# facebookresearch/esm

Measured on NVIDIA H100. Metric: sequences/sec ESM-2 650M L=1024 embedding extract, higher is better.
Workload: dtype f16 operands, f32 accumulate/residual/LayerNorm/softmax

## Files before the change

### esm_b200/csrc/api.cu

```cuda
#include "../../include/esmb200.h"

#include <cuda.h>
#include <cuda_runtime.h>
#include <stdio.h>
#include <stdlib.h>
#include <string.h>

#include <string>
#include <vector>

#include <mutex>

#include "attention8.cuh"
#include "attention_contact.cuh"
#include "attention_probs.cuh"
#include "common.cuh"
#include "elementwise.cuh"
#include "gemm2.cuh"
#include "tied_attention.cuh"

using namespace esmb200;

namespace {

thread_local std::string g_last_error;

int fail(int code, const std::string& msg) {
  g_last_error = msg;
  return code;
}

int fail_cuda(cudaError_t e, const char* what) {
  if (e == cudaErrorMemoryAllocation)
    return fail(ESMB200_ENOMEM, std::string("CUDA out of memory. (") + what + ")");
  return fail(ESMB200_ECUDA, std::string(what) + ": " + cudaGetErrorString(e));
}

#define CK(expr)                                        \
  do {                                                  \
    cudaError_t _e = (expr);                            \
    if (_e != cudaSuccess) return fail_cuda(_e, #expr); \
  } while (0)


enum ProfTag : int { T_LN1 = 0, T_QKV, T_ATTN, T_OUT, T_LN2, T_FC1, T_FC2, T_KEYBITS, T_EMBED, T_LN_F32, T_PROBS,
                     T_CONVERT, T_GEMM_OTHER, T_MEANPOOL, T_TIED_SCORES, T_TIED_SOFTMAX, T_TIED_PV, T_COUNT };
struct Profiler {
  std::mutex mu;
  bool on = false;
  std::vector<cudaEvent_t> ev;
  std::vector<int> tag;
  size_t used = 0;
  long long launches = 0;
};
Profiler g_prof;

struct ProfScope {
  cudaStream_t st;
  bool rec;
  size_t slot = 0;
  ProfScope(int tag, cudaStream_t s) : st(s), rec(false) {
    std::lock_guard<std::mutex> lk(g_prof.mu);
    ++g_prof.launches;
    if (g_prof.on && g_prof.used + 2 <= g_prof.ev.size()) {
      rec = true;
      slot = g_prof.used;
      g_prof.used += 2;
      g_prof.tag.push_back(tag);
      cudaEventRecord(g_prof.ev[slot], st);
    }
  }
  ~ProfScope() {
    if (rec) cudaEventRecord(g_prof.ev[slot + 1], st);
  }
};

typedef CUresult (*EncodeTiledFn)(CUtensorMap*, CUtensorMapDataType, cuuint32_t, void*, const cuuint64_t*,
                                  const cuuint64_t*, const cuuint32_t*, const cuuint32_t*, CUtensorMapInterleave,
                                  CUtensorMapSwizzle, CUtensorMapL2promotion, CUtensorMapFloatOOBfill);

EncodeTiledFn get_encode_fn() {
  static EncodeTiledFn fn = nullptr;
  if (fn) return fn;
  void* p = nullptr;
  cudaDriverEntryPointQueryResult qres;
  if (cudaGetDriverEntryPoint("cuTensorMapEncodeTiled", &p, cudaEnableDefault, &qres) != cudaSuccess ||
      qres != cudaDriverEntryPointSuccess)
    return nullptr;
  fn = reinterpret_cast<EncodeTiledFn>(p);
  return fn;
}

int make_tmap_2d(CUtensorMap* map, const void* ptr, int esize, uint64_t rows, uint64_t cols, uint64_t ld_elems,
                 uint32_t box_rows) {
  EncodeTiledFn enc = get_encode_fn();
  if (!enc) return fail(ESMB200_ECUDA, "cuTensorMapEncodeTiled entry point not available");
  if ((reinterpret_cast<uintptr_t>(ptr) & 15) != 0 || (ld_elems * esize) % 16 != 0)
    return fail(ESMB200_EINVAL, "TMA operand must be 16-byte aligned with a 16-byte multiple row pitch");
  cuuint64_t dims[2] = {cols, rows};
  cuuint64_t strides[1] = {ld_elems * (uint64_t)esize};
  cuuint32_t box[2] = {(cuuint32_t)(128 / esize), box_rows};
  cuuint32_t estr[2] = {1, 1};
  CUresult r = enc(map, esize == 2 ? CU_TENSOR_MAP_DATA_TYPE_FLOAT16 : CU_TENSOR_MAP_DATA_TYPE_FLOAT32, 2,
                   const_cast<void*>(ptr), dims, strides, box, estr,
                   CU_TENSOR_MAP_INTERLEAVE_NONE, CU_TENSOR_MAP_SWIZZLE_128B, CU_TENSOR_MAP_L2_PROMOTION_L2_256B,
                   CU_TENSOR_MAP_FLOAT_OOB_FILL_NONE);
  if (r != CUDA_SUCCESS) {
    char buf[160];
    snprintf(buf, sizeof buf, "cuTensorMapEncodeTiled failed (%d) rows=%llu cols=%llu ld=%llu box_rows=%u", (int)r,
             (unsigned long long)rows, (unsigned long long)cols, (unsigned long long)ld_elems, box_rows);
    return fail(ESMB200_ECUDA, buf);
  }
  return ESMB200_OK;
}

int make_tmap_f16(CUtensorMap* map, const void* ptr, uint64_t rows, uint64_t cols, uint64_t ld_elems,
                  uint32_t box_rows) {
  return make_tmap_2d(map, ptr, 2, rows, cols, ld_elems, box_rows);
}

inline int head_slots(int E, int H) { return (H > 0 && E / H > 64) ? 2 : 1; }

constexpr int kMaxDevices = 64;

int num_sms() {
  static int n[kMaxDevices] = {};
  int dev = 0;
  cudaGetDevice(&dev);
  if (dev < 0 || dev >= kMaxDevices) dev = 0;
  if (n[dev] == 0) cudaDeviceGetAttribute(&n[dev], cudaDevAttrMultiProcessorCount, dev);
  return n[dev];
}

int check_device() {
  static int ok[kMaxDevices] = {};
  int dev = 0;
  if (cudaGetDevice(&dev) != cudaSuccess) return fail(ESMB200_ECUDA, "no CUDA device");
  if (dev < 0 || dev >= kMaxDevices) return fail(ESMB200_ECUDA, "device ordinal out of range");
  if (ok[dev] == 0) {
    int major = 0;
    cudaDeviceGetAttribute(&major, cudaDevAttrComputeCapabilityMajor, dev);
    ok[dev] = (major == 9) ? 1 : -1;
  }
  if (ok[dev] < 0)
    return fail(ESMB200_ECUDA, "esmb200 requires an sm_90a (Hopper H100) device; there is no fallback path");
  return ESMB200_OK;
}

size_t align_up(size_t v, size_t a) { return (v + a - 1) / a * a; }

int launch_gemm(int epi, const CUtensorMap& ta, const CUtensorMap& tb, const GemmParams& p, cudaStream_t st,
                int tag = T_GEMM_OTHER, bool split = false) {
  ProfScope ps(tag, st);
  cudaError_t e;
  if (split) {
    if (p.K % 64 != 0) return fail(ESMB200_EINVAL, "fp32x3 precision needs K % 64 == 0");
    switch (epi) {
      case EPI_QKV_ROPE: e = launch_gemm2_epi<EPI_QKV_ROPE, true>(ta, tb, p, num_sms(), st); break;
      case EPI_BIAS_RESIDUAL: e = launch_gemm2_epi<EPI_BIAS_RESIDUAL, true>(ta, tb, p, num_sms(), st); break;
      case EPI_BIAS_GELU: e = launch_gemm2_epi<EPI_BIAS_GELU, true>(ta, tb, p, num_sms(), st); break;
      case EPI_BIAS_F32: e = launch_gemm2_epi<EPI_BIAS_F32, true>(ta, tb, p, num_sms(), st); break;
      case EPI_BIAS_GELU_F32: e = launch_gemm2_epi<EPI_BIAS_GELU_F32, true>(ta, tb, p, num_sms(), st); break;
      default: return fail(ESMB200_EINVAL, "unknown GEMM epilogue");
    }
    if (e != cudaSuccess) return fail_cuda(e, "gemm launch (fp32x3)");
    return ESMB200_OK;
  }
  switch (epi) {
    case EPI_QKV_ROPE: e = launch_gemm2_epi<EPI_QKV_ROPE>(ta, tb, p, num_sms(), st); break;
    case EPI_BIAS_RESIDUAL: e = launch_gemm2_epi<EPI_BIAS_RESIDUAL>(ta, tb, p, num_sms(), st); break;
    case EPI_BIAS_GELU: e = launch_gemm2_epi<EPI_BIAS_GELU>(ta, tb, p, num_sms(), st); break;
    case EPI_BIAS_F32: e = launch_gemm2_epi<EPI_BIAS_F32>(ta, tb, p, num_sms(), st); break;
    case EPI_BIAS_GELU_F32: e = launch_gemm2_epi<EPI_BIAS_GELU_F32>(ta, tb, p, num_sms(), st); break;
    default: return fail(ESMB200_EINVAL, "unknown GEMM epilogue");
  }
  if (e != cudaSuccess) return fail_cuda(e, "gemm launch");
  return ESMB200_OK;
}

struct AttnScratch {
  uint32_t* keybits;
  int* kvlen;
  float* row_max;
  float* row_sum;
  int words;
};

size_t attn_scratch_bytes(int B, int T, int H) {
  const int words = (int)align_up((size_t)(T + 31) / 32, 4);
  return align_up((size_t)B * words * 4, 256) + align_up((size_t)B * 4, 256) + 2 * align_up((size_t)B * H * T * 4, 256);
}

AttnScratch carve_attn_scratch(void* scratch, int B, int T, int H) {
  AttnScratch s;
  s.words = (int)align_up((size_t)(T + 31) / 32, 4);
  uint8_t* p = static_cast<uint8_t*>(scratch);
  s.keybits = reinterpret_cast<uint32_t*>(p);
  p += align_up((size_t)B * s.words * 4, 256);
  s.kvlen = reinterpret_cast<int*>(p);
  p += align_up((size_t)B * 4, 256);
  s.row_max = reinterpret_cast<float*>(p);
  p += align_up((size_t)B * H * T * 4, 256);
  s.row_sum = reinterpret_cast<float*>(p);
  return s;
}

int run_key_bits(const uint8_t* pad_mask, const AttnScratch& s, int B, int T, cudaStream_t st) {
  const int wpb = 4;
  ProfScope ps(T_KEYBITS, st);
  key_bits_kernel<<<(B + wpb - 1) / wpb, wpb * 32, 0, st>>>(pad_mask, s.keybits, s.kvlen, B, T, s.words);
  CK(cudaGetLastError());
  return ESMB200_OK;
}

struct ContactLayer {
  const float* w;
  const uint8_t* keep;
  float* acc;
  float* row_part;
  float* col_part;
  int lo, S;
};

int run_attention(const void* qkv, void* ctx, float* probs, long long probs_batch_stride, int attn_flags,
                  const AttnScratch& s, int B, int T, int H, cudaStream_t st, bool split = false,
                  const ContactLayer* contact = nullptr, int slots = 1) {
  const int E = H * 64 * slots;
  if (slots == 2 && split) return fail(ESMB200_EINVAL, "head_dim > 64: fp32x3 precision is not available");
  const uint64_t qcols = (uint64_t)(split ? 6 : 3) * E;
  CUtensorMap tq;
  int rc = make_tmap_f16(&tq, qkv, (uint64_t)B * T, qcols, qcols, 128);
  if (rc) return rc;
  AttnParams ap;
  ap.B = B; ap.T = T; ap.H = H; ap.E = E;
  ap.lo_off = split ? 3 * E : 0;
  ap.slots = slots;
  ap.keybits = s.keybits; ap.kvlen = s.kvlen; ap.words = s.words;
  ap.ctx = static_cast<__half*>(ctx);
  ap.row_max = probs ? s.row_max : nullptr;
  ap.row_sum = probs ? s.row_sum : nullptr;
  cudaError_t e;
  {
    CUtensorMap tkv;
    rc = make_tmap_f16(&tkv, qkv, (uint64_t)B * T, qcols, qcols, attn8_cfg::BLOCK_KV);
    if (rc) return rc;
    ProfScope ps(T_ATTN, st);
    e = launch_attention_fwd(tq, tkv, ap, st);
  }
  if (e != cudaSuccess) return fail_cuda(e, "attention launch");
  if (probs && contact && !split) {
    if (B > 65535) return fail(ESMB200_EINVAL, "return_contacts: B must be <= 65535");
    ContactFuseParams cp;
    cp.B = B; cp.T = T; cp.H = H; cp.E = E; cp.slots = slots;
    cp.keybits = s.keybits; cp.kvlen = s.kvlen; cp.words = s.words;
    cp.row_max = s.row_max; cp.row_sum = s.row_sum; cp.probs = probs;
    cp.batch_stride = probs_batch_stride > 0 ? probs_batch_stride : (long long)H * T * T;
    cp.zero_pad_rows = attn_flags & 1;
    cp.w = contact->w; cp.keep = contact->keep; cp.acc = contact->acc;
    cp.row_part = contact->row_part; cp.col_part = contact->col_part; cp.lo = contact->lo; cp.S = contact->S;
    {
      ProfScope ps(T_PROBS, st);
      e = launch_attention_probs_contact(tq, cp, st);
    }
    if (e != cudaSuccess) return fail_cuda(e, "attention probs+contact launch");
    return ESMB200_OK;
  }
  if (probs) {
    if ((size_t)B * H > 65535) return fail(ESMB200_EINVAL, "need_head_weights: B*H must be <= 65535");
    ProbsParams pp;
    pp.B = B; pp.T = T; pp.H = H; pp.E = E;
    pp.keybits = s.keybits; pp.kvlen = s.kvlen; pp.words = s.words;
    pp.row_max = s.row_max; pp.row_sum = s.row_sum; pp.probs = probs;
    pp.batch_stride = probs_batch_stride > 0 ? probs_batch_stride : (long long)H * T * T;
    pp.zero_pad_rows = attn_flags & 1;
    pp.lo_off = split ? 3 * E : 0;
    pp.slots = slots;
    {
      ProfScope ps(T_PROBS, st);
      e = launch_attention_probs(tq, pp, st);
    }
    if (e != cudaSuccess) return fail_cuda(e, "attention probs launch");
  }
  return ESMB200_OK;
}

}

struct esmb200_layer {
  int E, H, F;
  int d;
  int slots;
  int Ea;
  float q_scale;
  int split;
  float eps;
  const float *ln1_w, *ln1_b, *ln2_w, *ln2_b, *out_b, *fc1_b, *fc2_b;
  __half* w_qkv;
  __half* w_out;
  __half* w_fc1;
  __half* w_fc2;
  float* b_qkv;
  CUtensorMap tm_qkv, tm_out, tm_fc1, tm_fc2;
};

extern "C" {

int esmb200_abi_version(void) { return ESMB200_ABI_VERSION; }

const char* esmb200_last_error(void) { return g_last_error.c_str(); }

int esmb200_convert_f16(const float* src, void* dst, size_t n, void* stream) {
  if (n == 0) return ESMB200_OK;
  cudaStream_t st = static_cast<cudaStream_t>(stream);
  size_t blocks = (n + 255) / 256;
  if (blocks > (size_t)num_sms() * 16) blocks = (size_t)num_sms() * 16;
  ProfScope ps(T_CONVERT, st);
  convert_f32_f16_kernel<<<(unsigned)blocks, 256, 0, st>>>(src, static_cast<__half*>(dst), n);
  CK(cudaGetLastError());
  return ESMB200_OK;
}

int esmb200_layer_destroy(esmb200_layer* L) {
  if (!L) return ESMB200_OK;
  cudaFree(L->w_qkv);
  cudaFree(L->w_out);
  cudaFree(L->w_fc1);
  cudaFree(L->w_fc2);
  cudaFree(L->b_qkv);
  delete L;
  return ESMB200_OK;
}

int esmb200_layer_create(const esmb200_layer_weights* w, void* stream, esmb200_layer** out) {
  if (!w || !out) return fail(ESMB200_EINVAL, "null argument");
  int rc = check_device();
  if (rc) return rc;
  const int E = w->embed_dim, H = w->num_heads, F = w->ffn_dim;
  if (E <= 0 || H <= 0 || E % H != 0) return fail(ESMB200_EINVAL, "embed_dim must be a positive multiple of num_heads");
  const int d = w->head_dim > 0 ? w->head_dim : E / H;
  if (d * H != E || d > 128 || d % 2 != 0)
    return fail(ESMB200_EINVAL, "esmb200 supports even head_dim <= 128 (every ESM-2 model, MSA Transformer)");
  if (E % 16 != 0) return fail(ESMB200_EINVAL, "embed_dim must be a multiple of 16");
  const bool has_ffn = w->fc1_weight != nullptr;
  if (has_ffn && (F <= 0 || F % 64 != 0)) return fail(ESMB200_EINVAL, "ffn_dim must be a positive multiple of 64");
  cudaStream_t st = static_cast<cudaStream_t>(stream);
  esmb200_layer* L = new esmb200_layer();
  memset(static_cast<void*>(L), 0, sizeof(*L));
  const int slots = head_slots(E, H);
  const int Ea = 64 * slots * H;
  L->E = E; L->H = H; L->F = has_ffn ? F : 0; L->d = d; L->slots = slots; L->Ea = Ea; L->eps = w->ln_eps;
  L->q_scale = 1.0f / sqrtf((float)d);
  L->ln1_w = w->ln1_weight; L->ln1_b = w->ln1_bias; L->ln2_w = w->ln2_weight; L->ln2_b = w->ln2_bias;
  L->out_b = w->out_bias; L->fc1_b = w->fc1_bias; L->fc2_b = w->fc2_bias;
  if (w->precision != 0 && w->precision != 1) {
    delete L;
    return fail(ESMB200_EINVAL, "precision must be 0 (fp16 operands) or 1 (fp32x3: fp16 hi|lo operands)");
  }
  const int split = w->precision;
  if (split && slots == 2) {
    delete L;
    return fail(ESMB200_EINVAL, "fp32x3 precision is not available for head_dim > 64");
  }
  if (split && (E % 64 != 0 || (has_ffn && F % 64 != 0))) {
    delete L;
    return fail(ESMB200_EINVAL, "fp32x3 precision needs embed_dim % 64 == 0 (all ESM-2 models except 35M)");
  }
  L->split = split;
  const size_t pf = split ? 2 : 1;
  const size_t EaE = (size_t)Ea * E, EF = (size_t)E * F;
  cudaError_t e;
#define ALLOC(ptr, bytes)                                              \
  if ((e = cudaMalloc(reinterpret_cast<void**>(&(ptr)), (bytes))) != cudaSuccess) { \
    esmb200_layer_destroy(L);                                          \
    return fail_cuda(e, "cudaMalloc(packed weights)");                 \
  }
  ALLOC(L->w_qkv, 3 * EaE * 2 * pf);
  ALLOC(L->w_out, EaE * 2 * pf);
  if (has_ffn) {
    ALLOC(L->w_fc1, EF * 2 * pf);
    ALLOC(L->w_fc2, EF * 2 * pf);
  }
  ALLOC(L->b_qkv, (size_t)3 * Ea * 4);
#undef ALLOC
  auto convert = [&](const float* src, __half* dst, size_t rows, int K) -> int {
    if (!split) return esmb200_convert_f16(src, dst, rows * (size_t)K, stream);
    size_t blocks = (rows * (size_t)K + 255) / 256;
    if (blocks > (size_t)num_sms() * 16) blocks = (size_t)num_sms() * 16;
    ProfScope ps(T_CONVERT, st);
    convert_f32_split_kernel<<<(unsigned)blocks, 256, 0, st>>>(src, dst, rows, K);
    cudaError_t ce = cudaGetLastError();
    return ce == cudaSuccess ? ESMB200_OK : fail_cuda(ce, "convert_f32_split");
  };
  if (d == 64 && !split) {
    rc = esmb200_convert_f16(w->q_weight, L->w_qkv, EaE, stream);
    if (!rc) rc = esmb200_convert_f16(w->k_weight, L->w_qkv + EaE, EaE, stream);
    if (!rc) rc = esmb200_convert_f16(w->v_weight, L->w_qkv + 2 * EaE, EaE, stream);
    if (!rc) rc = esmb200_convert_f16(w->out_weight, L->w_out, EaE, stream);
    if (!rc) {
      e = cudaMemcpyAsync(L->b_qkv, w->q_bias, (size_t)E * 4, cudaMemcpyDeviceToDevice, st);
      if (e == cudaSuccess) e = cudaMemcpyAsync(L->b_qkv + E, w->k_bias, (size_t)E * 4, cudaMemcpyDeviceToDevice, st);
      if (e == cudaSuccess) e = cudaMemcpyAsync(L->b_qkv + 2 * E, w->v_bias, (size_t)E * 4, cudaMemcpyDeviceToDevice, st);
      if (e != cudaSuccess) rc = fail_cuda(e, "bias pack");
    }
  } else {
    e = cudaMemsetAsync(L->w_qkv, 0, 3 * EaE * 2 * pf, st);
    if (e == cudaSuccess) e = cudaMemsetAsync(L->w_out, 0, EaE * 2 * pf, st);
    if (e == cudaSuccess) e = cudaMemsetAsync(L->b_qkv, 0, (size_t)3 * Ea * 4, st);
    if (e != cudaSuccess) rc = fail_cuda(e, "memset(packed weights)");
    const float* ws3[3] = {w->q_weight, w->k_weight, w->v_weight};
    const float* bs3[3] = {w->q_bias, w->k_bias, w->v_bias};
    const unsigned blocks = (unsigned)(((size_t)E * E + 255) / 256);
    for (int s3 = 0; s3 < 3 && !rc; ++s3) {
      ProfScope ps(T_CONVERT, st);
      pack_head_rows_kernel<<<blocks, 256, 0, st>>>(ws3[s3], bs3[s3], L->w_qkv + (size_t)s3 * EaE * pf, L->b_qkv + s3 * Ea,
                                                    E, d, split);
      if ((e = cudaGetLastError()) != cudaSuccess) rc = fail_cuda(e, "pack_head_rows");
    }
    if (!rc) {
      ProfScope ps(T_CONVERT, st);
      pack_head_cols_kernel<<<blocks, 256, 0, st>>>(w->out_weight, L->w_out, E, Ea, d, split);
      if ((e = cudaGetLastError()) != cudaSuccess) rc = fail_cuda(e, "pack_head_cols");
    }
  }
  if (!rc && has_ffn) rc = convert(w->fc1_weight, L->w_fc1, F, E);
  if (!rc && has_ffn) rc = convert(w->fc2_weight, L->w_fc2, E, F);
  const uint32_t wbox = gemm2_cfg::HALF_N;
  if (!rc) rc = make_tmap_f16(&L->tm_qkv, L->w_qkv, 3 * (uint64_t)Ea, pf * E, pf * E, wbox);
  if (!rc) rc = make_tmap_f16(&L->tm_out, L->w_out, E, pf * Ea, pf * Ea, wbox);
  if (!rc && has_ffn) rc = make_tmap_f16(&L->tm_fc1, L->w_fc1, F, pf * E, pf * E, wbox);
  if (!rc && has_ffn) rc = make_tmap_f16(&L->tm_fc2, L->w_fc2, E, pf * F, pf * F, wbox);
  if (rc) {
    esmb200_layer_destroy(L);
    return rc;
  }
  *out = L;
  return ESMB200_OK;
}

size_t esmb200_attention_scratch_bytes(int32_t B, int32_t T) {
  return attn_scratch_bytes(B, T, 64);
}

size_t esmb200_workspace_bytes(int32_t E, int32_t H, int32_t F, int32_t B, int32_t T, int32_t precision) {
  const size_t M = (size_t)B * T, Ea = (size_t)64 * head_slots(E, H) * H, pf = precision ? 2 : 1;
  const size_t a = align_up(M * E * 2 * pf, 1024);
  const size_t big_qkv_ctx = align_up(M * 3 * Ea * 2 * pf, 1024) + align_up(M * Ea * 2 * pf, 1024);
  const size_t big_h = align_up(M * F * 2 * pf, 1024);
  const size_t big = big_qkv_ctx > big_h ? big_qkv_ctx : big_h;
  return a + big + attn_scratch_bytes(B, T, H) + 1024;
}

namespace {
struct Workspace {
  __half* xn;
  __half* qkv;
  __half* ctx;
  __half* h;
  AttnScratch as;
};

int carve_workspace(Workspace* ws, void* workspace, size_t bytes, int E, int H, int F, int B, int T, int split) {
  if (bytes < esmb200_workspace_bytes(E, H, F, B, T, split)) return fail(ESMB200_EWORKSPACE, "workspace too small");
  const size_t M = (size_t)B * T, Ea = (size_t)64 * head_slots(E, H) * H, pf = split ? 2 : 1;
  uint8_t* p = reinterpret_cast<uint8_t*>(align_up(reinterpret_cast<uintptr_t>(workspace), 1024));
  ws->xn = reinterpret_cast<__half*>(p);
  p += align_up(M * E * 2 * pf, 1024);
  ws->qkv = reinterpret_cast<__half*>(p);
  ws->h = reinterpret_cast<__half*>(p);
  ws->ctx = reinterpret_cast<__half*>(p + align_up(M * 3 * Ea * 2 * pf, 1024));
  const size_t big_qkv_ctx = align_up(M * 3 * Ea * 2 * pf, 1024) + align_up(M * Ea * 2 * pf, 1024);
  const size_t big_h = align_up(M * F * 2 * pf, 1024);
  p += big_qkv_ctx > big_h ? big_qkv_ctx : big_h;
  ws->as = carve_attn_scratch(p, B, T, H);
  return ESMB200_OK;
}

struct ActMaps {
  CUtensorMap xn, ctx, h;
};

int layer_forward_impl(esmb200_layer* L, float* x, int B, int T, const float* rope_cos, const float* rope_sin,
                       float* attn_probs, long long attn_batch_stride, int attn_flags, const Workspace& ws,
                       const ActMaps& am, cudaStream_t st, const ContactLayer* contact = nullptr) {
  const int E = L->E, F = L->F, H = L->H, Ea = L->Ea;
  const int M = B * T;
  const bool split = L->split != 0;
  cudaError_t e = cudaSuccess;
  {
    ProfScope ps(T_LN1, st);
    e = split ? launch_layernorm<2>(x, L->ln1_w, L->ln1_b, ws.xn, M, E, L->eps, st)
              : launch_layernorm<1>(x, L->ln1_w, L->ln1_b, ws.xn, M, E, L->eps, st);
  }
  if (e != cudaSuccess) return fail_cuda(e, "layernorm1");
  GemmParams g;
  memset(&g, 0, sizeof g);
  g.M = M; g.N = 3 * Ea; g.K = E; g.bias = L->b_qkv; g.out = ws.qkv; g.ldo = 3 * Ea;
  g.rope_cos = rope_cos; g.rope_sin = rope_sin; g.T = T; g.E = Ea; g.q_scale = L->q_scale;
  g.lo_col_off = 3 * Ea;
  g.rope_ld = 32 * L->slots;
  int rc = launch_gemm(EPI_QKV_ROPE, am.xn, L->tm_qkv, g, st, T_QKV, split);
  if (rc) return rc;
  rc = run_attention(ws.qkv, ws.ctx, attn_probs, attn_batch_stride, attn_flags, ws.as, B, T, H, st, split, contact,
                     L->slots);
  if (rc) return rc;
  memset(&g, 0, sizeof g);
  g.M = M; g.N = E; g.K = Ea; g.bias = L->out_b; g.out = x; g.ldo = E;
  rc = launch_gemm(EPI_BIAS_RESIDUAL, am.ctx, L->tm_out, g, st, T_OUT, split);
  if (rc) return rc;
  {
    ProfScope ps(T_LN2, st);
    e = split ? launch_layernorm<2>(x, L->ln2_w, L->ln2_b, ws.xn, M, E, L->eps, st)
              : launch_layernorm<1>(x, L->ln2_w, L->ln2_b, ws.xn, M, E, L->eps, st);
  }
  if (e != cudaSuccess) return fail_cuda(e, "layernorm2");
  memset(&g, 0, sizeof g);
  g.M = M; g.N = F; g.K = E; g.bias = L->fc1_b; g.out = ws.h; g.ldo = F; g.lo_col_off = F;
  rc = launch_gemm(EPI_BIAS_GELU, am.xn, L->tm_fc1, g, st, T_FC1, split);
  if (rc) return rc;
  memset(&g, 0, sizeof g);
  g.M = M; g.N = E; g.K = F; g.bias = L->fc2_b; g.out = x; g.ldo = E;
  rc = launch_gemm(EPI_BIAS_RESIDUAL, am.h, L->tm_fc2, g, st, T_FC2, split);
  return rc;
}

int make_act_maps(ActMaps* am, const Workspace& ws, int E, int H, int F, int M, int split = 0) {
  const uint64_t Ea = (uint64_t)64 * head_slots(E, H) * H, pf = split ? 2 : 1;
  int rc = make_tmap_f16(&am->xn, ws.xn, M, pf * E, pf * E, gemm2_cfg::BOX_M);
  if (!rc) rc = make_tmap_f16(&am->ctx, ws.ctx, M, pf * Ea, pf * Ea, gemm2_cfg::BOX_M);
  if (!rc) rc = make_tmap_f16(&am->h, ws.h, M, pf * F, pf * F, gemm2_cfg::BOX_M);
  return rc;
}
}

int esmb200_stack_forward(esmb200_layer* const* layers, int32_t n_layers, float* x, const uint8_t* pad_mask,
                          int32_t B, int32_t T, const float* rope_cos, const float* rope_sin,
                          float* const* repr_out, float* const* attn_out, int64_t attn_batch_stride,
                          int32_t attn_flags, const esmb200_contact_job* contact, void* workspace,
                          size_t workspace_bytes, void* stream) {
  if (!layers || n_layers <= 0 || !x || !rope_cos || !rope_sin || !workspace)
    return fail(ESMB200_EINVAL, "null argument");
  if (contact) {
    if (!attn_out) return fail(ESMB200_EINVAL, "a contact job needs attn_out for every layer");
    for (int i = 0; i < n_layers; ++i)
      if (!attn_out[i]) return fail(ESMB200_EINVAL, "a contact job needs attn_out for every layer");
    if (!contact->weights || !contact->acc || !contact->row_part || !contact->col_part || contact->lo < 0 ||
        contact->hi > T || contact->hi <= contact->lo)
      return fail(ESMB200_EINVAL, "bad contact job");
  }
  if (B <= 0 || T <= 0) return fail(ESMB200_EINVAL, "empty batch");
  if ((long long)B * T > 0x7fffffffLL / 8) return fail(ESMB200_EINVAL, "B*T too large for one call; split the batch");
  int rc = check_device();
  if (rc) return rc;
  cudaStream_t st = static_cast<cudaStream_t>(stream);
  const int E = layers[0]->E, F = layers[0]->F, H = layers[0]->H;
  if (F <= 0) return fail(ESMB200_EINVAL, "attention-only layers belong to esmb200_axial_stack_forward");
  for (int i = 1; i < n_layers; ++i)
    if (layers[i]->E != E || layers[i]->F != F || layers[i]->H != H || layers[i]->split != layers[0]->split)
      return fail(ESMB200_EINVAL, "layers of one stack must share E, H, F and precision");
  const int split = layers[0]->split;
  Workspace ws;
  rc = carve_workspace(&ws, workspace, workspace_bytes, E, H, F, B, T, split);
  if (rc) return rc;
  ActMaps am;
  rc = make_act_maps(&am, ws, E, H, F, B * T, split);
  if (rc) return rc;
  rc = run_key_bits(pad_mask, ws.as, B, T, st);
  if (rc) return rc;
  const int nt128 = (T + 127) / 128;
  for (int i = 0; i < n_layers; ++i) {
    ContactLayer cl;
    if (contact) {
      const int S = contact->hi - contact->lo;
      const size_t part = (size_t)B * H * nt128 * S;
      cl.w = contact->weights + (size_t)i * H; cl.keep = contact->keep; cl.acc = contact->acc;
      cl.row_part = contact->row_part + (size_t)i * 4 * part; cl.col_part = contact->col_part + (size_t)i * 4 * part;
      cl.lo = contact->lo; cl.S = S;
    }
    rc = layer_forward_impl(layers[i], x, B, T, rope_cos, rope_sin, attn_out ? attn_out[i] : nullptr, attn_batch_stride,
                            attn_flags, ws, am, st, contact ? &cl : nullptr);
    if (rc) return rc;
    if (repr_out && repr_out[i])
      CK(cudaMemcpyAsync(repr_out[i], x, (size_t)B * T * E * 4, cudaMemcpyDeviceToDevice, st));
  }
  return ESMB200_OK;
}

int esmb200_layer_forward(esmb200_layer* layer, float* x, const uint8_t* pad_mask, int32_t B, int32_t T,
                          const float* rope_cos, const float* rope_sin, float* attn_probs, void* workspace,
                          size_t workspace_bytes, void* stream) {
  if (!layer) return fail(ESMB200_EINVAL, "null layer");
  float* attn_arr[1] = {attn_probs};
  esmb200_layer* arr[1] = {layer};
  return esmb200_stack_forward(arr, 1, x, pad_mask, B, T, rope_cos, rope_sin, nullptr, attn_probs ? attn_arr : nullptr,
                               0, 0, nullptr, workspace, workspace_bytes, stream);
}

int esmb200_embed_tokens(const int64_t* tokens, const float* table, float* x, int32_t B, int32_t T, int32_t E,
                         int32_t padding_idx, int32_t mask_idx, int32_t token_dropout, void* stream) {
  if (!tokens || !table || !x) return fail(ESMB200_EINVAL, "null argument");
  if (B <= 0 || B > 65535 || T <= 0 || E % 4 != 0) return fail(ESMB200_EINVAL, "bad shape");
  ProfScope ps(T_EMBED, static_cast<cudaStream_t>(stream));
  int chunks = (8 * num_sms() + B - 1) / B;
  if (chunks > (T + 3) / 4) chunks = (T + 3) / 4;
  if (chunks < 1) chunks = 1;
  embed_tokens_kernel<<<dim3(chunks, B), 256, 0, static_cast<cudaStream_t>(stream)>>>(tokens, table, x, T, E, padding_idx,
                                                                                     mask_idx, token_dropout);
  CK(cudaGetLastError());
  return ESMB200_OK;
}

int esmb200_layernorm(const float* x, const float* weight, const float* bias, float* out, int32_t M, int32_t E,
                      float eps, void* stream) {
  if (!x || !weight || !bias || !out) return fail(ESMB200_EINVAL, "null argument");
  ProfScope ps(T_LN_F32, static_cast<cudaStream_t>(stream));
  cudaError_t e = launch_layernorm<0>(x, weight, bias, out, M, E, eps, static_cast<cudaStream_t>(stream));
  if (e != cudaSuccess) return fail_cuda(e, "layernorm");
  return ESMB200_OK;
}

int esmb200_layernorm_f16(const float* x, const float* weight, const float* bias, void* out, int32_t M, int32_t E,
                          float eps, void* stream) {
  if (!x || !weight || !bias || !out) return fail(ESMB200_EINVAL, "null argument");
  ProfScope ps(T_LN1, static_cast<cudaStream_t>(stream));
  cudaError_t e = launch_layernorm<1>(x, weight, bias, out, M, E, eps, static_cast<cudaStream_t>(stream));
  if (e != cudaSuccess) return fail_cuda(e, "layernorm_f16");
  return ESMB200_OK;
}

int esmb200_gemm_f16(int32_t epilogue, const void* a, const void* w, const float* bias, void* out, int32_t M,
                     int32_t N, int32_t K, const float* rope_cos, const float* rope_sin, int32_t T, int32_t E,
                     void* stream) {
  if (!a || !w || !bias || !out) return fail(ESMB200_EINVAL, "null argument");
  const bool f16_out = (epilogue == EPI_QKV_ROPE || epilogue == EPI_BIAS_GELU);
  if (M <= 0 || N <= 0 || K <= 0 || K % 8 != 0 || N % (f16_out ? 64 : 32) != 0)
    return fail(ESMB200_EINVAL, "gemm needs K % 8 == 0 and N % 64 == 0 (fp16 output) / N % 32 == 0 (fp32 output)");
  int rc = check_device();
  if (rc) return rc;
  if (epilogue == EPI_QKV_ROPE && (!rope_cos || !rope_sin || T <= 0 || E <= 0 || E % 64 != 0 || N != 3 * E))
    return fail(ESMB200_EINVAL, "qkv epilogue needs rope tables, T and N == 3E");
  CUtensorMap ta, tb;
  rc = make_tmap_f16(&ta, a, M, K, K, gemm2_cfg::BOX_M);
  if (!rc) rc = make_tmap_f16(&tb, w, N, K, K, gemm2_cfg::HALF_N);
  if (rc) return rc;
  GemmParams g;
  memset(&g, 0, sizeof g);
  g.M = M; g.N = N; g.K = K; g.bias = bias; g.out = out; g.ldo = N;
  g.rope_cos = rope_cos; g.rope_sin = rope_sin; g.T = T; g.E = E; g.q_scale = 0.125f;
  return launch_gemm(epilogue, ta, tb, g, static_cast<cudaStream_t>(stream));
}

int esmb200_layernorm_split(const float* x, const float* weight, const float* bias, void* out, int32_t M, int32_t E,
                            float eps, void* stream) {
  if (!x || !weight || !bias || !out) return fail(ESMB200_EINVAL, "null argument");
  ProfScope ps(T_LN1, static_cast<cudaStream_t>(stream));
  cudaError_t e = launch_layernorm<2>(x, weight, bias, out, M, E, eps, static_cast<cudaStream_t>(stream));
  if (e != cudaSuccess) return fail_cuda(e, "layernorm_split");
  return ESMB200_OK;
}

int esmb200_convert_split(const float* src, void* dst, int64_t rows, int32_t K, void* stream) {
  if (!src || !dst) return fail(ESMB200_EINVAL, "null argument");
  if (rows <= 0 || K <= 0) return ESMB200_OK;
  cudaStream_t st = static_cast<cudaStream_t>(stream);
  size_t blocks = ((size_t)rows * K + 255) / 256;
  if (blocks > (size_t)num_sms() * 16) blocks = (size_t)num_sms() * 16;
  ProfScope ps(T_CONVERT, st);
  convert_f32_split_kernel<<<(unsigned)blocks, 256, 0, st>>>(src, static_cast<__half*>(dst), (size_t)rows, K);
  CK(cudaGetLastError());
  return ESMB200_OK;
}

int esmb200_gemm_split(int32_t epilogue, const void* a, const void* w, const float* bias, void* out, int32_t M,
                       int32_t N, int32_t K, const float* rope_cos, const float* rope_sin, int32_t T, int32_t E,
                       void* stream) {
  if (!a || !w || !bias || !out) return fail(ESMB200_EINVAL, "null argument");
  const bool f16_out = (epilogue == EPI_QKV_ROPE || epilogue == EPI_BIAS_GELU);
  if (M <= 0 || N <= 0 || K <= 0 || K % 64 != 0 || N % (f16_out ? 64 : 32) != 0)
    return fail(ESMB200_EINVAL, "split gemm needs K % 64 == 0 and N % 64 == 0 (fp16 output) / N % 32 == 0 (fp32 output)");
  if (epilogue < 0 || epilogue > EPI_BIAS_GELU_F32) return fail(ESMB200_EINVAL, "unknown GEMM epilogue");
  int rc = check_device();
  if (rc) return rc;
  if (epilogue == EPI_QKV_ROPE && (!rope_cos || !rope_sin || T <= 0 || E <= 0 || E % 64 != 0 || N != 3 * E))
    return fail(ESMB200_EINVAL, "qkv epilogue needs rope tables, T and N == 3E");
  CUtensorMap ta, tb;
  rc = make_tmap_f16(&ta, a, M, 2 * (uint64_t)K, 2 * (uint64_t)K, gemm2_cfg::BOX_M);
  if (!rc) rc = make_tmap_f16(&tb, w, N, 2 * (uint64_t)K, 2 * (uint64_t)K, gemm2_cfg::HALF_N);
  if (rc) return rc;
  GemmParams g;
  memset(&g, 0, sizeof g);
  g.M = M; g.N = N; g.K = K; g.bias = bias; g.out = out; g.ldo = N; g.lo_col_off = N;
  g.rope_cos = rope_cos; g.rope_sin = rope_sin; g.T = T; g.E = E; g.q_scale = 0.125f;
  return launch_gemm(epilogue, ta, tb, g, static_cast<cudaStream_t>(stream), T_GEMM_OTHER, true);
}

int esmb200_attention_split(const void* qkv, const uint8_t* pad_mask, void* ctx, float* attn_probs, int32_t B, int32_t T,
                            int32_t H, void* scratch, void* stream) {
  if (!qkv || !ctx || !scratch) return fail(ESMB200_EINVAL, "null argument");
  if (B <= 0 || T <= 0 || H <= 0 || H > 64) return fail(ESMB200_EINVAL, "bad shape");
  int rc = check_device();
  if (rc) return rc;
  cudaStream_t st = static_cast<cudaStream_t>(stream);
  AttnScratch s = carve_attn_scratch(scratch, B, T, H);
  rc = run_key_bits(pad_mask, s, B, T, st);
  if (rc) return rc;
  return run_attention(qkv, ctx, attn_probs, 0, 0, s, B, T, H, st, true);
}

int esmb200_gemm_qkv_f16(const void* a, const void* w, const float* bias, void* out, int32_t M, int32_t E, float q_scale,
                         const float* rope_cos, const float* rope_sin, int32_t T, void* stream) {
  if (!a || !w || !bias || !out) return fail(ESMB200_EINVAL, "null argument");
  if (M <= 0 || E <= 0 || E % 64 != 0) return fail(ESMB200_EINVAL, "qkv gemm needs E % 64 == 0");
  if ((rope_cos == nullptr) != (rope_sin == nullptr) || (rope_cos && T <= 0))
    return fail(ESMB200_EINVAL, "rope tables must be given together with T, or not at all");
  int rc = check_device();
  if (rc) return rc;
  CUtensorMap ta, tb;
  rc = make_tmap_f16(&ta, a, M, E, E, gemm2_cfg::BOX_M);
  if (!rc) rc = make_tmap_f16(&tb, w, 3 * (uint64_t)E, E, E, gemm2_cfg::HALF_N);
  if (rc) return rc;
  GemmParams g;
  memset(&g, 0, sizeof g);
  g.M = M; g.N = 3 * E; g.K = E; g.bias = bias; g.out = out; g.ldo = 3 * E;
  g.rope_cos = rope_cos; g.rope_sin = rope_sin; g.T = T > 0 ? T : 1; g.E = E; g.q_scale = q_scale;
  return launch_gemm(EPI_QKV_ROPE, ta, tb, g, static_cast<cudaStream_t>(stream));
}

int esmb200_attention(const void* qkv, const uint8_t* pad_mask, void* ctx, float* attn_probs, int32_t B, int32_t T,
                      int32_t H, void* scratch, void* stream) {
  if (!qkv || !ctx || !scratch) return fail(ESMB200_EINVAL, "null argument");
  if (B <= 0 || T <= 0 || H <= 0 || H > 64) return fail(ESMB200_EINVAL, "bad shape");
  int rc = check_device();
  if (rc) return rc;
  cudaStream_t st = static_cast<cudaStream_t>(stream);
  AttnScratch s = carve_attn_scratch(scratch, B, T, H);
  rc = run_key_bits(pad_mask, s, B, T, st);
  if (rc) return rc;
  return run_attention(qkv, ctx, attn_probs, 0, 0, s, B, T, H, st);
}

int esmb200_attention128(const void* qkv, const uint8_t* pad_mask, void* ctx, float* attn_probs, int32_t B, int32_t T,
                         int32_t H, void* scratch, void* stream) {
  if (!qkv || !ctx || !scratch) return fail(ESMB200_EINVAL, "null argument");
  if (B <= 0 || T <= 0 || H <= 0 || H > 64) return fail(ESMB200_EINVAL, "bad shape");
  int rc = check_device();
  if (rc) return rc;
  cudaStream_t st = static_cast<cudaStream_t>(stream);
  AttnScratch s = carve_attn_scratch(scratch, B, T, H);
  rc = run_key_bits(pad_mask, s, B, T, st);
  if (rc) return rc;
  return run_attention(qkv, ctx, attn_probs, 0, 0, s, B, T, H, st, false, nullptr, 2);
}

size_t esmb200_tied_row_attention_scratch_bytes(int32_t B, int32_t C, int32_t H) {
  const size_t Cp = align_up((size_t)C, 64);
  return align_up((size_t)H * B * C * C * 4, 1024) + align_up((size_t)H * B * C * Cp * 2, 1024) + 2048;
}

static int tied_row_impl(const void* qkv, const uint8_t* key_pad, long long key_pad_stride, void* ctx,
                         float* attn_probs, int32_t B, int32_t R, int32_t C, int32_t H, void* scratch,
                         size_t scratch_bytes, void* stream) {
  if (!qkv || !ctx || !scratch) return fail(ESMB200_EINVAL, "null argument");
  if (B <= 0 || R <= 0 || C <= 0 || H <= 0 || H > 64 || (long long)B * H > 65535)
    return fail(ESMB200_EINVAL, "bad shape");
  if (C > TIED_MAX_C) return fail(ESMB200_EINVAL, "tied row attention supports at most 1024 alignment columns");
  if (scratch_bytes < esmb200_tied_row_attention_scratch_bytes(B, C, H))
    return fail(ESMB200_EWORKSPACE, "tied row attention scratch too small");
  int rc = check_device();
  if (rc) return rc;
  cudaStream_t st = static_cast<cudaStream_t>(stream);
  const int E = H * 64;
  const size_t Cp = align_up((size_t)C, 64);
  uint8_t* sp = reinterpret_cast<uint8_t*>(align_up(reinterpret_cast<uintptr_t>(scratch), 1024));
  TiedParams tp;
  tp.B = B; tp.R = R; tp.C = C; tp.H = H; tp.E = E; tp.Cp = (int)Cp;
  tp.S = attn_probs ? attn_probs : reinterpret_cast<float*>(sp);
  tp.P = reinterpret_cast<__half*>(sp + align_up((size_t)H * B * C * C * 4, 1024));
  tp.ctx = static_cast<__half*>(ctx);
  tp.key_pad = key_pad;
  tp.key_pad_stride = key_pad_stride;
  tp.write_probs = attn_probs ? 1 : 0;
  const uint64_t rows = (uint64_t)B * R * C;
  CUtensorMap tq, tk, tv, tpm;
  if ((rc = make_tmap_f16(&tq, qkv, rows, (uint64_t)3 * E, (uint64_t)3 * E, tied_cfg::S_BM))) return rc;
  if ((rc = make_tmap_f16(&tk, qkv, rows, (uint64_t)3 * E, (uint64_t)3 * E, tied_cfg::S_BN))) return rc;
  if ((rc = make_tmap_f16(&tv, qkv, rows, (uint64_t)3 * E, (uint64_t)3 * E, 64))) return rc;
  if ((rc = make_tmap_f16(&tpm, tp.P, (uint64_t)H * B * C, Cp, Cp, tied_cfg::V_BM))) return rc;
  cudaError_t e;
  {
    ProfScope ps(T_TIED_SCORES, st);
    e = launch_tied_scores(tq, tk, tp, st);
  }
  if (e != cudaSuccess) return fail_cuda(e, "tied scores launch");
  {
    ProfScope ps(T_TIED_SOFTMAX, st);
    e = launch_tied_softmax(tp, st);
  }
  if (e != cudaSuccess) return fail_cuda(e, "tied softmax launch");
  {
    ProfScope ps(T_TIED_PV, st);
    e = launch_tied_pv(tpm, tv, tp, st);
  }
  if (e != cudaSuccess) return fail_cuda(e, "tied update launch");
  return ESMB200_OK;
}

int esmb200_tied_row_attention(const void* qkv, const uint8_t* key_pad, void* ctx, float* attn_probs, int32_t B,
                               int32_t R, int32_t C, int32_t H, void* scratch, size_t scratch_bytes, void* stream) {
  return tied_row_impl(qkv, key_pad, C, ctx, attn_probs, B, R, C, H, scratch, scratch_bytes, stream);
}

int esmb200_column_attention(const void* qkv, const uint8_t* pad_mask, void* ctx, int32_t B, int32_t R, int32_t C,
                             int32_t H, void* scratch, void* stream) {
  if (!qkv || !ctx || !scratch) return fail(ESMB200_EINVAL, "null argument");
  if (B <= 0 || R <= 0 || C <= 0 || H <= 0 || H > 64) return fail(ESMB200_EINVAL, "bad shape");
  int rc = check_device();
  if (rc) return rc;
  cudaStream_t st = static_cast<cudaStream_t>(stream);
  const int E = H * 64;
  const int S = B * C;
  AttnScratch s = carve_attn_scratch(scratch, S, R, H);
  rc = run_key_bits(pad_mask, s, S, R, st);
  if (rc) return rc;
  CUtensorMap tq, tkv;
  const uint64_t wide = (uint64_t)C * 3 * E;
  if ((rc = make_tmap_f16(&tq, qkv, (uint64_t)B * R, wide, wide, attn8_cfg::BLOCK_Q))) return rc;
  if ((rc = make_tmap_f16(&tkv, qkv, (uint64_t)B * R, wide, wide, attn8_cfg::BLOCK_KV))) return rc;
  AttnParams ap;
  ap.B = S; ap.T = R; ap.H = H; ap.E = E;
  ap.keybits = s.keybits; ap.kvlen = s.kvlen; ap.words = s.words;
  ap.ctx = static_cast<__half*>(ctx);
  ap.row_max = nullptr; ap.row_sum = nullptr;
  ap.cols = C;
  cudaError_t e;
  {
    ProfScope ps(T_ATTN, st);
    e = launch_attention_fwd(tq, tkv, ap, st);
  }
  if (e != cudaSuccess) return fail_cuda(e, "column attention launch");
  return ESMB200_OK;
}


size_t esmb200_axial_workspace_bytes(int32_t E, int32_t F, int32_t B, int32_t R, int32_t C) {
  return esmb200_workspace_bytes(E, E / 64, F, B * C, R, 0) + esmb200_tied_row_attention_scratch_bytes(B, C, E / 64) + 1024;
}

int esmb200_axial_stack_forward(esmb200_layer* const* row_layers, esmb200_layer* const* col_layers, int32_t n_layers,
                                float* x, const uint8_t* pad_mask, const uint8_t* col_pad_mask, int32_t B, int32_t R,
                                int32_t C, float* const* row_attn_out, void* workspace, size_t workspace_bytes,
                                void* stream) {
  if (!row_layers || !col_layers || n_layers <= 0 || !x || !workspace) return fail(ESMB200_EINVAL, "null argument");
  if (B <= 0 || R <= 0 || C <= 0) return fail(ESMB200_EINVAL, "empty alignment");
  if ((pad_mask == nullptr) != (col_pad_mask == nullptr))
    return fail(ESMB200_EINVAL, "pad_mask [B,R,C] and col_pad_mask [B,C,R] must be given together");
  if ((long long)B * R * C > 0x7fffffffLL / 8) return fail(ESMB200_EINVAL, "B*R*C too large for one call");
  int rc = check_device();
  if (rc) return rc;
  cudaStream_t st = static_cast<cudaStream_t>(stream);
  const int E = col_layers[0]->E, F = col_layers[0]->F, H = col_layers[0]->H;
  if (F <= 0) return fail(ESMB200_EINVAL, "col_layers carry the feed-forward weights");
  for (int i = 0; i < n_layers; ++i)
    if (row_layers[i]->E != E || col_layers[i]->E != E || col_layers[i]->F != F)
      return fail(ESMB200_EINVAL, "layers of one stack must share E and F");
  if (workspace_bytes < esmb200_axial_workspace_bytes(E, F, B, R, C))
    return fail(ESMB200_EWORKSPACE, "workspace too small");
  const int M = B * R * C;
  Workspace ws;
  if (E != 64 * H) return fail(ESMB200_EINVAL, "the MSA axial path needs head_dim 64");
  for (int i = 0; i < n_layers; ++i)
    if (row_layers[i]->split || col_layers[i]->split)
      return fail(ESMB200_EINVAL, "the MSA axial path runs with fp16 operands only (precision 0)");
  const size_t base_bytes = esmb200_workspace_bytes(E, H, F, B * C, R, 0);
  rc = carve_workspace(&ws, workspace, base_bytes, E, H, F, B * C, R, 0);
  if (rc) return rc;
  uint8_t* tied_scratch = reinterpret_cast<uint8_t*>(align_up(reinterpret_cast<uintptr_t>(workspace), 1024)) + base_bytes;
  const size_t tied_bytes = esmb200_tied_row_attention_scratch_bytes(B, C, H);
  ActMaps am;
  rc = make_act_maps(&am, ws, E, H, F, M);
  if (rc) return rc;
  rc = run_key_bits(col_pad_mask, ws.as, B * C, R, st);
  if (rc) return rc;
  CUtensorMap tcq, tckv;
  const uint64_t wide = (uint64_t)C * 3 * E;
  if ((rc = make_tmap_f16(&tcq, ws.qkv, (uint64_t)B * R, wide, wide, attn8_cfg::BLOCK_Q))) return rc;
  if ((rc = make_tmap_f16(&tckv, ws.qkv, (uint64_t)B * R, wide, wide, attn8_cfg::BLOCK_KV))) return rc;
  const float row_scale = 0.125f / sqrtf((float)R);
  cudaError_t e;
  GemmParams g;
  for (int i = 0; i < n_layers; ++i) {
    esmb200_layer* L = row_layers[i];
    {
      ProfScope ps(T_LN1, st);
      e = launch_layernorm<1>(x, L->ln1_w, L->ln1_b, ws.xn, M, E, L->eps, st);
    }
    if (e != cudaSuccess) return fail_cuda(e, "row layernorm");
    memset(&g, 0, sizeof g);
    g.M = M; g.N = 3 * E; g.K = E; g.bias = L->b_qkv; g.out = ws.qkv; g.ldo = 3 * E;
    g.T = 1; g.E = E; g.q_scale = row_scale;
    rc = launch_gemm(EPI_QKV_ROPE, am.xn, L->tm_qkv, g, st, T_QKV);
    if (rc) return rc;
    if (pad_mask) {
      ProfScope ps(T_KEYBITS, st);
      zero_q_at_pads_kernel<<<(M + 7) / 8, 256, 0, st>>>(ws.qkv, pad_mask, M, E);
      CK(cudaGetLastError());
    }
    rc = tied_row_impl(ws.qkv, pad_mask, (long long)R * C, ws.ctx, row_attn_out ? row_attn_out[i] : nullptr, B, R, C, H,
                       tied_scratch, tied_bytes, stream);
    if (rc) return rc;
    memset(&g, 0, sizeof g);
    g.M = M; g.N = E; g.K = E; g.bias = L->out_b; g.out = x; g.ldo = E;
    rc = launch_gemm(EPI_BIAS_RESIDUAL, am.ctx, L->tm_out, g, st, T_OUT);
    if (rc) return rc;
    L = col_layers[i];
    {
      ProfScope ps(T_LN1, st);
      e = launch_layernorm<1>(x, L->ln1_w, L->ln1_b, ws.xn, M, E, L->eps, st);
    }
    if (e != cudaSuccess) return fail_cuda(e, "column layernorm");
    memset(&g, 0, sizeof g);
    g.M = M; g.N = 3 * E; g.K = E; g.bias = L->b_qkv; g.out = ws.qkv; g.ldo = 3 * E;
    g.T = 1; g.E = E; g.q_scale = 0.125f;
    rc = launch_gemm(EPI_QKV_ROPE, am.xn, L->tm_qkv, g, st, T_QKV);
    if (rc) return rc;
    {
      AttnParams ap;
      ap.B = B * C; ap.T = R; ap.H = H; ap.E = E;
      ap.keybits = ws.as.keybits; ap.kvlen = ws.as.kvlen; ap.words = ws.as.words;
      ap.ctx = ws.ctx; ap.row_max = nullptr; ap.row_sum = nullptr; ap.cols = C;
      ProfScope ps(T_ATTN, st);
      e = launch_attention_fwd(tcq, tckv, ap, st);
    }
    if (e != cudaSuccess) return fail_cuda(e, "column attention launch");
    memset(&g, 0, sizeof g);
    g.M = M; g.N = E; g.K = E; g.bias = L->out_b; g.out = x; g.ldo = E;
    rc = launch_gemm(EPI_BIAS_RESIDUAL, am.ctx, L->tm_out, g, st, T_OUT);
    if (rc) return rc;
    {
      ProfScope ps(T_LN2, st);
      e = launch_layernorm<1>(x, L->ln2_w, L->ln2_b, ws.xn, M, E, L->eps, st);
    }
    if (e != cudaSuccess) return fail_cuda(e, "ffn layernorm");
    memset(&g, 0, sizeof g);
    g.M = M; g.N = F; g.K = E; g.bias = L->fc1_b; g.out = ws.h; g.ldo = F;
    rc = launch_gemm(EPI_BIAS_GELU, am.xn, L->tm_fc1, g, st, T_FC1);
    if (rc) return rc;
    memset(&g, 0, sizeof g);
    g.M = M; g.N = E; g.K = F; g.bias = L->fc2_b; g.out = x; g.ldo = E;
    rc = launch_gemm(EPI_BIAS_RESIDUAL, am.h, L->tm_fc2, g, st, T_FC2);
    if (rc) return rc;
  }
  return ESMB200_OK;
}



int esmb200_msa_embed(const int64_t* tokens, const float* embed_table, const float* pos_table, const float* msa_pos,
                      int32_t msa_pos_dim, const float* ln_weight, const float* ln_bias, float eps, float* x,
                      int32_t B, int32_t R, int32_t C, int32_t E, int32_t padding_idx, void* stream) {
  if (!tokens || !embed_table || !pos_table || !ln_weight || !ln_bias || !x) return fail(ESMB200_EINVAL, "null argument");
  if (B <= 0 || R <= 0 || C <= 0 || E <= 0 || E % 4 != 0 || E > 20 * 128) return fail(ESMB200_EINVAL, "bad shape");
  if (msa_pos && msa_pos_dim != E && msa_pos_dim != 1)
    return fail(ESMB200_EINVAL, "msa_position_embedding width must be E or 1");
  cudaStream_t st = static_cast<cudaStream_t>(stream);
  ProfScope ps(T_EMBED, st);
  const size_t smem = (size_t)C * sizeof(int);
  const int grid = B * R;
  if (E <= 4 * 128)
    msa_embed_kernel<4><<<grid, 256, smem, st>>>(tokens, embed_table, pos_table, msa_pos, msa_pos_dim, ln_weight,
                                                  ln_bias, eps, x, R, C, E, padding_idx);
  else if (E <= 10 * 128)
    msa_embed_kernel<10><<<grid, 256, smem, st>>>(tokens, embed_table, pos_table, msa_pos, msa_pos_dim, ln_weight,
                                                   ln_bias, eps, x, R, C, E, padding_idx);
  else
    msa_embed_kernel<20><<<grid, 256, smem, st>>>(tokens, embed_table, pos_table, msa_pos, msa_pos_dim, ln_weight,
                                                   ln_bias, eps, x, R, C, E, padding_idx);
  CK(cudaGetLastError());
  return ESMB200_OK;
}


int esmb200_contact_accumulate(const float* attn, int64_t batch_stride, const float* w, const uint8_t* keep, float* acc,
                               float* row_sum, float* col_part, int32_t B, int32_t H, int32_t T, int32_t lo, int32_t hi,
                               void* stream) {
  if (!attn || !w || !acc || !row_sum || !col_part) return fail(ESMB200_EINVAL, "null argument");
  const int S = hi - lo;
  if (B <= 0 || H <= 0 || T <= 0 || lo < 0 || hi > T || S <= 0 || B > 65535) return fail(ESMB200_EINVAL, "bad shape");
  if (S > 1024) return fail(ESMB200_EINVAL, "contact head supports at most 1024 positions");
  cudaStream_t st = static_cast<cudaStream_t>(stream);
  ProfScope ps(T_PROBS, st);
  const size_t smem = (size_t)8 * S * sizeof(float);
  dim3 grid((S + 15) / 16, B);
  if (S <= 512)
    contact_accumulate_kernel<2, 16, 2><<<grid, 256, smem, st>>>(attn, batch_stride, w, keep, acc, row_sum, col_part, H, T,
                                                                  lo, S);
  else
    contact_accumulate_kernel<2, 32, 1><<<grid, 256, smem, st>>>(attn, batch_stride, w, keep, acc, row_sum, col_part, H, T,
                                                                  lo, S);
  CK(cudaGetLastError());
  return ESMB200_OK;
}

int esmb200_contact_finalize(const float* acc, const float* u, const float* a1, const float* bias, float* out, int32_t B,
                             int32_t C, int32_t S, void* stream) {
  if (!acc || !u || !a1 || !out) return fail(ESMB200_EINVAL, "null argument");
  if (B <= 0 || C <= 0 || S <= 0 || B > 65535) return fail(ESMB200_EINVAL, "bad shape");
  cudaStream_t st = static_cast<cudaStream_t>(stream);
  ProfScope ps(T_PROBS, st);
  dim3 grid((S + 63) / 64, (S + 63) / 64, B);
  contact_finalize_kernel<<<grid, 256, 0, st>>>(acc, u, a1, bias, out, C, S);
  CK(cudaGetLastError());
  return ESMB200_OK;
}


int esmb200_mean_pool(const float* x, const int32_t* lengths, float* out, int32_t B, int32_t T, int32_t E,
                      void* stream) {
  if (!x || !lengths || !out) return fail(ESMB200_EINVAL, "null argument");
  if (B <= 0 || T < 2 || E <= 0 || B > 65535) return fail(ESMB200_EINVAL, "bad shape");
  cudaStream_t st = static_cast<cudaStream_t>(stream);
  ProfScope ps(T_MEANPOOL, st);
  if (E % 4 != 0) return fail(ESMB200_EINVAL, "mean_pool needs E % 4 == 0");
  dim3 grid((E + 127) / 128, B);
  mean_pool_kernel<<<grid, 256, 0, st>>>(x, lengths, out, T, E);
  CK(cudaGetLastError());
  return ESMB200_OK;
}


int esmb200_set_option(const char* name, int32_t value) {
  if (!name) return fail(ESMB200_EINVAL, "null option name");
  if (!strcmp(name, "pdl") && (value == 0 || value == 1)) { pdl_flag() = value; return ESMB200_OK; }
  return fail(ESMB200_EINVAL, std::string("unknown option or value: ") + name);
}

long long esmb200_launch_count(void) {
  std::lock_guard<std::mutex> lk(g_prof.mu);
  return g_prof.launches;
}

int esmb200_profile_enable(int32_t max_launches) {
  std::lock_guard<std::mutex> lk(g_prof.mu);
  for (cudaEvent_t e : g_prof.ev) cudaEventDestroy(e);
  g_prof.ev.clear();
  g_prof.tag.clear();
  g_prof.used = 0;
  g_prof.on = max_launches > 0;
  for (int i = 0; i < 2 * max_launches; ++i) {
    cudaEvent_t e;
    CK(cudaEventCreate(&e));
    g_prof.ev.push_back(e);
  }
  return ESMB200_OK;
}

int esmb200_profile_read(int32_t* tags, float* ms, int32_t max_records) {
  std::lock_guard<std::mutex> lk(g_prof.mu);
  const int n = (int)(g_prof.used / 2);
  int out = 0;
  for (int i = 0; i < n && out < max_records; ++i, ++out) {
    CK(cudaEventSynchronize(g_prof.ev[2 * i + 1]));
    float t = 0.f;
    CK(cudaEventElapsedTime(&t, g_prof.ev[2 * i], g_prof.ev[2 * i + 1]));
    tags[out] = g_prof.tag[i];
    ms[out] = t;
  }
  g_prof.used = 0;
  g_prof.tag.clear();
  return out;
}

}
```

### esm_b200/csrc/common.cuh

```cuda
#pragma once

#include <cuda.h>
#include <cuda_fp16.h>
#include <cuda_runtime.h>
#include <stdint.h>
#include <stdio.h>
#include <stdlib.h>

#ifndef ESMB200_WATCHDOG
#define ESMB200_WATCHDOG 1
#endif

namespace esmb200 {

constexpr uint32_t kWarp = 32;

__device__ __forceinline__ uint32_t smem_u32(const void* p) {
  return static_cast<uint32_t>(__cvta_generic_to_shared(p));
}

__device__ __forceinline__ uint32_t lane_id() {
  uint32_t r;
  asm volatile("mov.u32 %0, %%laneid;" : "=r"(r));
  return r;
}

__device__ __forceinline__ bool elect_one() {
  uint32_t pred = 0;
  asm volatile(
      "{\n\t"
      ".reg .pred P1;\n\t"
      "elect.sync _|P1, 0xffffffff;\n\t"
      "selp.u32 %0, 1, 0, P1;\n\t"
      "}\n"
      : "=r"(pred));
  return pred != 0;
}

__device__ __forceinline__ void mbar_init(uint64_t* bar, uint32_t count) {
  asm volatile("mbarrier.init.shared::cta.b64 [%0], %1;" ::"r"(smem_u32(bar)), "r"(count) : "memory");
}

__device__ __forceinline__ void fence_barrier_init() {
  asm volatile("fence.mbarrier_init.release.cluster;" ::: "memory");
}

__device__ __forceinline__ void fence_proxy_async_smem() {
  asm volatile("fence.proxy.async.shared::cta;" ::: "memory");
}

__device__ __forceinline__ void mbar_arrive(uint64_t* bar) {
  asm volatile("mbarrier.arrive.shared::cta.b64 _, [%0];" ::"r"(smem_u32(bar)) : "memory");
}

__device__ __forceinline__ void mbar_arrive_expect_tx(uint64_t* bar, uint32_t bytes) {
  asm volatile("mbarrier.arrive.expect_tx.shared::cta.b64 _, [%0], %1;" ::"r"(smem_u32(bar)), "r"(bytes)
               : "memory");
}

__device__ __forceinline__ bool mbar_try_wait(uint64_t* bar, uint32_t parity) {
  uint32_t ok;
  asm volatile(
      "{\n\t"
      ".reg .pred p;\n\t"
      "mbarrier.try_wait.parity.shared::cta.b64 p, [%1], %2;\n\t"
      "selp.u32 %0, 1, 0, p;\n\t"
      "}\n"
      : "=r"(ok)
      : "r"(smem_u32(bar)), "r"(parity)
      : "memory");
  return ok != 0;
}

__device__ __forceinline__ void mbar_wait(uint64_t* bar, uint32_t parity) {
  if (mbar_try_wait(bar, parity)) return;
#if ESMB200_WATCHDOG
  uint32_t polls = 0;
  while (!mbar_try_wait(bar, parity)) {
    if (++polls == (1u << 26)) {
      printf("esmb200: mbarrier watchdog block=(%d,%d,%d) thread=%d bar=%u parity=%u\n", blockIdx.x, blockIdx.y,
             blockIdx.z, threadIdx.x, smem_u32(bar), parity);
      __trap();
    }
  }
#else
  while (!mbar_try_wait(bar, parity)) {
  }
#endif
}


__device__ __forceinline__ void mbar_wait_relaxed(uint64_t* bar, uint32_t parity) {
  if (mbar_try_wait(bar, parity)) return;
#if ESMB200_WATCHDOG
  uint32_t polls = 0;
#endif
  while (!mbar_try_wait(bar, parity)) {
    __nanosleep(200);
#if ESMB200_WATCHDOG
    if (++polls == (1u << 24)) {
      printf("esmb200: mbarrier watchdog (relaxed) block=(%d,%d,%d) thread=%d bar=%u parity=%u\n", blockIdx.x, blockIdx.y,
             blockIdx.z, threadIdx.x, smem_u32(bar), parity);
      __trap();
    }
#endif
  }
}

__device__ __forceinline__ void tma_prefetch_desc(const CUtensorMap* map) {
  asm volatile("prefetch.tensormap [%0];" ::"l"(reinterpret_cast<uint64_t>(map)) : "memory");
}

__device__ __forceinline__ void tma_load_2d(void* smem_dst, const CUtensorMap* map, uint64_t* bar, int32_t c0,
                                            int32_t c1) {
  asm volatile(
      "cp.async.bulk.tensor.2d.shared::cluster.global.mbarrier::complete_tx::bytes [%0], [%1, {%3, %4}], [%2];"
      :
      : "r"(smem_u32(smem_dst)), "l"(reinterpret_cast<uint64_t>(map)), "r"(smem_u32(bar)), "r"(c0), "r"(c1)
      : "memory");
}

__device__ __forceinline__ void tma_load_2d_addr(uint32_t smem_dst, const CUtensorMap* map, uint32_t bar, int32_t c0,
                                                 int32_t c1) {
  asm volatile(
      "cp.async.bulk.tensor.2d.shared::cluster.global.mbarrier::complete_tx::bytes [%0], [%1, {%3, %4}], [%2];"
      :
      : "r"(smem_dst), "l"(reinterpret_cast<uint64_t>(map)), "r"(bar), "r"(c0), "r"(c1)
      : "memory");
}
__device__ __forceinline__ void mbar_arrive_expect_tx_addr(uint32_t bar, uint32_t bytes) {
  asm volatile("mbarrier.arrive.expect_tx.shared::cta.b64 _, [%0], %1;" ::"r"(bar), "r"(bytes) : "memory");
}

__device__ __forceinline__ void tma_load_2d_hint(void* smem_dst, const CUtensorMap* map, uint64_t* bar, int32_t c0,
                                                 int32_t c1, uint64_t policy) {
  asm volatile(
      "cp.async.bulk.tensor.2d.shared::cluster.global.mbarrier::complete_tx::bytes.L2::cache_hint [%0], [%1, {%3, "
      "%4}], [%2], %5;"
      :
      : "r"(smem_u32(smem_dst)), "l"(reinterpret_cast<uint64_t>(map)), "r"(smem_u32(bar)), "r"(c0), "r"(c1),
        "l"(policy)
      : "memory");
}

__device__ __forceinline__ uint64_t l2_policy_evict_last() {
  uint64_t p;
  asm volatile("createpolicy.fractional.L2::evict_last.b64 %0, 1.0;" : "=l"(p));
  return p;
}
__device__ __forceinline__ uint64_t l2_policy_evict_first() {
  uint64_t p;
  asm volatile("createpolicy.fractional.L2::evict_first.b64 %0, 1.0;" : "=l"(p));
  return p;
}

__device__ __forceinline__ void mma16816(float (&d)[4], const uint32_t (&a)[4], uint32_t b0, uint32_t b1) {
  asm volatile(
      "mma.sync.aligned.m16n8k16.row.col.f32.f16.f16.f32 {%0, %1, %2, %3}, {%4, %5, %6, %7}, {%8, %9}, "
      "{%0, %1, %2, %3};"
      : "+f"(d[0]), "+f"(d[1]), "+f"(d[2]), "+f"(d[3])
      : "r"(a[0]), "r"(a[1]), "r"(a[2]), "r"(a[3]), "r"(b0), "r"(b1));
}

__device__ __forceinline__ void ldsm_x4(uint32_t addr, uint32_t (&r)[4]) {
  asm volatile("ldmatrix.sync.aligned.m8n8.x4.shared.b16 {%0, %1, %2, %3}, [%4];"
               : "=r"(r[0]), "=r"(r[1]), "=r"(r[2]), "=r"(r[3])
               : "r"(addr));
}
__device__ __forceinline__ void ldsm_x4_t(uint32_t addr, uint32_t (&r)[4]) {
  asm volatile("ldmatrix.sync.aligned.m8n8.x4.trans.shared.b16 {%0, %1, %2, %3}, [%4];"
               : "=r"(r[0]), "=r"(r[1]), "=r"(r[2]), "=r"(r[3])
               : "r"(addr));
}

__device__ __forceinline__ uint32_t sw128(uint32_t base, uint32_t row, uint32_t chunk) {
  return base + row * 128u + ((chunk ^ (row & 7u)) << 4);
}

__device__ __forceinline__ void ldsm_a(uint32_t base, uint32_t r0, uint32_t kk, uint32_t (&a)[4]) {
  const uint32_t l = lane_id();
  ldsm_x4(sw128(base, r0 + (l & 15u), 2u * kk + (l >> 4)), a);
}
__device__ __forceinline__ void ldsm_b(uint32_t base, uint32_t n0, uint32_t kk, uint32_t (&b)[4]) {
  const uint32_t l = lane_id();
  ldsm_x4(sw128(base, n0 + (l & 7u) + ((l >> 4) << 3), 2u * kk + ((l >> 3) & 1u)), b);
}
__device__ __forceinline__ void ldsm_bt(uint32_t base, uint32_t kk, uint32_t n0, uint32_t (&b)[4]) {
  const uint32_t l = lane_id();
  ldsm_x4_t(sw128(base, 16u * kk + (l & 15u), n0 / 8u + (l >> 4)), b);
}

__device__ __forceinline__ uint64_t wgmma_desc_sw128(uint32_t smem_addr) {
  uint64_t d = 0;
  d |= static_cast<uint64_t>((smem_addr & 0x3FFFFu) >> 4);
  d |= static_cast<uint64_t>(1) << 16;
  d |= static_cast<uint64_t>(1024 >> 4) << 32;
  d |= static_cast<uint64_t>(1) << 62;
  return d;
}

__device__ __forceinline__ void wgmma_fence() { asm volatile("wgmma.fence.sync.aligned;" ::: "memory"); }
__device__ __forceinline__ void wgmma_commit() { asm volatile("wgmma.commit_group.sync.aligned;" ::: "memory"); }
template <int N>
__device__ __forceinline__ void wgmma_wait() {
  asm volatile("wgmma.wait_group.sync.aligned %0;" ::"n"(N) : "memory");
}
template <int N>
__device__ __forceinline__ void reg_fence_f(float (&r)[N]) {
#pragma unroll
  for (int i = 0; i < N; ++i) asm volatile("" : "+f"(r[i])::"memory");
}

__device__ __forceinline__ void wgmma_m64n256k16(float (&d)[128], uint64_t da, uint64_t db, int scale_d) {
  asm volatile(
      "{\n.reg .pred p;\nsetp.ne.b32 p, %130, 0;\n"
      "wgmma.mma_async.sync.aligned.m64n256k16.f32.f16.f16 "
      "{%0, %1, %2, %3, %4, %5, %6, %7, %8, %9, %10, %11, %12, %13, %14, %15, "
      "%16, %17, %18, %19, %20, %21, %22, %23, %24, %25, %26, %27, %28, %29, %30, %31, "
      "%32, %33, %34, %35, %36, %37, %38, %39, %40, %41, %42, %43, %44, %45, %46, %47, "
      "%48, %49, %50, %51, %52, %53, %54, %55, %56, %57, %58, %59, %60, %61, %62, %63, "
      "%64, %65, %66, %67, %68, %69, %70, %71, %72, %73, %74, %75, %76, %77, %78, %79, "
      "%80, %81, %82, %83, %84, %85, %86, %87, %88, %89, %90, %91, %92, %93, %94, %95, "
      "%96, %97, %98, %99, %100, %101, %102, %103, %104, %105, %106, %107, %108, %109, %110, %111, "
      "%112, %113, %114, %115, %116, %117, %118, %119, %120, %121, %122, %123, %124, %125, %126, %127}, "
      "%128, %129, p, 1, 1, 0, 0;\n}\n"
      : "+f"(d[0]), "+f"(d[1]), "+f"(d[2]), "+f"(d[3]), "+f"(d[4]), "+f"(d[5]), "+f"(d[6]), "+f"(d[7]),
        "+f"(d[8]), "+f"(d[9]), "+f"(d[10]), "+f"(d[11]), "+f"(d[12]), "+f"(d[13]), "+f"(d[14]), "+f"(d[15]),
        "+f"(d[16]), "+f"(d[17]), "+f"(d[18]), "+f"(d[19]), "+f"(d[20]), "+f"(d[21]), "+f"(d[22]), "+f"(d[23]),
        "+f"(d[24]), "+f"(d[25]), "+f"(d[26]), "+f"(d[27]), "+f"(d[28]), "+f"(d[29]), "+f"(d[30]), "+f"(d[31]),
        "+f"(d[32]), "+f"(d[33]), "+f"(d[34]), "+f"(d[35]), "+f"(d[36]), "+f"(d[37]), "+f"(d[38]), "+f"(d[39]),
        "+f"(d[40]), "+f"(d[41]), "+f"(d[42]), "+f"(d[43]), "+f"(d[44]), "+f"(d[45]), "+f"(d[46]), "+f"(d[47]),
        "+f"(d[48]), "+f"(d[49]), "+f"(d[50]), "+f"(d[51]), "+f"(d[52]), "+f"(d[53]), "+f"(d[54]), "+f"(d[55]),
        "+f"(d[56]), "+f"(d[57]), "+f"(d[58]), "+f"(d[59]), "+f"(d[60]), "+f"(d[61]), "+f"(d[62]), "+f"(d[63]),
        "+f"(d[64]), "+f"(d[65]), "+f"(d[66]), "+f"(d[67]), "+f"(d[68]), "+f"(d[69]), "+f"(d[70]), "+f"(d[71]),
        "+f"(d[72]), "+f"(d[73]), "+f"(d[74]), "+f"(d[75]), "+f"(d[76]), "+f"(d[77]), "+f"(d[78]), "+f"(d[79]),
        "+f"(d[80]), "+f"(d[81]), "+f"(d[82]), "+f"(d[83]), "+f"(d[84]), "+f"(d[85]), "+f"(d[86]), "+f"(d[87]),
        "+f"(d[88]), "+f"(d[89]), "+f"(d[90]), "+f"(d[91]), "+f"(d[92]), "+f"(d[93]), "+f"(d[94]), "+f"(d[95]),
        "+f"(d[96]), "+f"(d[97]), "+f"(d[98]), "+f"(d[99]), "+f"(d[100]), "+f"(d[101]), "+f"(d[102]), "+f"(d[103]),
        "+f"(d[104]), "+f"(d[105]), "+f"(d[106]), "+f"(d[107]), "+f"(d[108]), "+f"(d[109]), "+f"(d[110]), "+f"(d[111]),
        "+f"(d[112]), "+f"(d[113]), "+f"(d[114]), "+f"(d[115]), "+f"(d[116]), "+f"(d[117]), "+f"(d[118]), "+f"(d[119]),
        "+f"(d[120]), "+f"(d[121]), "+f"(d[122]), "+f"(d[123]), "+f"(d[124]), "+f"(d[125]), "+f"(d[126]), "+f"(d[127])
      : "l"(da), "l"(db), "r"(scale_d));
}

template <uint32_t R>
__device__ __forceinline__ void setmaxnreg_dec() { asm volatile("setmaxnreg.dec.sync.aligned.u32 %0;" ::"n"(R)); }
template <uint32_t R>
__device__ __forceinline__ void setmaxnreg_inc() { asm volatile("setmaxnreg.inc.sync.aligned.u32 %0;" ::"n"(R)); }

__device__ __forceinline__ void tma_store_2d(const CUtensorMap* map, const void* smem_src, int32_t c0, int32_t c1) {
  asm volatile("cp.async.bulk.tensor.2d.global.shared::cta.bulk_group [%0, {%2, %3}], [%1];" ::"l"(
                   reinterpret_cast<uint64_t>(map)),
               "r"(smem_u32(smem_src)), "r"(c0), "r"(c1)
               : "memory");
}
__device__ __forceinline__ void tma_reduce_add_2d(const CUtensorMap* map, const void* smem_src, int32_t c0,
                                                  int32_t c1) {
  asm volatile("cp.reduce.async.bulk.tensor.2d.global.shared::cta.add.tile.bulk_group [%0, {%2, %3}], [%1];" ::"l"(
                   reinterpret_cast<uint64_t>(map)),
               "r"(smem_u32(smem_src)), "r"(c0), "r"(c1)
               : "memory");
}
__device__ __forceinline__ void tma_store_commit() { asm volatile("cp.async.bulk.commit_group;" ::: "memory"); }
template <int N>
__device__ __forceinline__ void tma_store_wait_read() {
  asm volatile("cp.async.bulk.wait_group.read %0;" ::"n"(N) : "memory");
}
__device__ __forceinline__ void tma_store_wait_all() { asm volatile("cp.async.bulk.wait_group 0;" ::: "memory"); }

__device__ __forceinline__ void pdl_wait() { asm volatile("griddepcontrol.wait;" ::: "memory"); }
__device__ __forceinline__ void pdl_launch_dependents() { asm volatile("griddepcontrol.launch_dependents;" ::: "memory"); }

inline int& pdl_flag() {
  static int flag = -1;
  return flag;
}
inline bool pdl_enabled() {
  int& f = pdl_flag();
  if (f < 0) {
    const char* e = getenv("ESMB200_PDL");
    f = (e && e[0] == '1') ? 1 : 0;
  }
  return f != 0;
}

template <typename... KArgs, typename... Args>
inline cudaError_t launch_pdl(void (*kernel)(KArgs...), dim3 grid, dim3 block, size_t smem, cudaStream_t stream,
                              Args&&... args) {
  cudaLaunchConfig_t cfg = {};
  cfg.gridDim = grid;
  cfg.blockDim = block;
  cfg.dynamicSmemBytes = smem;
  cfg.stream = stream;
  cudaLaunchAttribute attr[1];
  attr[0].id = cudaLaunchAttributeProgrammaticStreamSerialization;
  attr[0].val.programmaticStreamSerializationAllowed = 1;
  cfg.attrs = attr;
  cfg.numAttrs = pdl_enabled() ? 1 : 0;
  return cudaLaunchKernelEx(&cfg, kernel, KArgs(args)...);
}

__device__ __forceinline__ uint32_t pack_half2(float lo, float hi) {
  __half2 h = __floats2half2_rn(lo, hi);
  return *reinterpret_cast<uint32_t*>(&h);
}

__device__ __forceinline__ void fma2(float& d0, float& d1, float a0, float a1, float b0, float b1, float c0, float c1) {
  d0 = fmaf(a0, b0, c0);
  d1 = fmaf(a1, b1, c1);
}
__device__ __forceinline__ void add2(float& d0, float& d1, float a0, float a1, float b0, float b1) {
  d0 = a0 + b0;
  d1 = a1 + b1;
}
__device__ __forceinline__ void mul2(float& d0, float& d1, float a0, float a1, float b0, float b1) {
  d0 = a0 * b0;
  d1 = a1 * b1;
}

__device__ __forceinline__ float ex2_approx(float x) {
  float y;
  asm("ex2.approx.ftz.f32 %0, %1;" : "=f"(y) : "f"(x));
  return y;
}

__device__ __forceinline__ float warp_sum(float v) {
#pragma unroll
  for (int o = 16; o > 0; o >>= 1) v += __shfl_xor_sync(0xffffffffu, v, o);
  return v;
}

__device__ __forceinline__ void named_bar_sync(uint32_t id, uint32_t nthreads) {
  asm volatile("bar.sync %0, %1;" ::"r"(id), "r"(nthreads) : "memory");
}

}
```

### esm_b200/csrc/gemm2.cuh

```cuda
#pragma once

#include "gemm_common.cuh"

namespace esmb200 {

namespace gemm2_cfg {
constexpr int BLOCK_M = 128;
constexpr int BLOCK_N = 256;
constexpr int HALF_N = 128;
constexpr int BLOCK_K = 64;
constexpr int STAGES = 4;
constexpr int A_STAGE_BYTES = BLOCK_M * BLOCK_K * 2;
constexpr int B_STAGE_BYTES = BLOCK_N * BLOCK_K * 2;
constexpr int STAGE_BYTES = A_STAGE_BYTES + B_STAGE_BYTES;
constexpr int BOX_M = 128;
constexpr int NUM_THREADS = 384;
constexpr int SMEM_BYTES = STAGES * STAGE_BYTES + 1024 + 256;
}

template <int EPI, bool SPLIT = false>
__global__ void __launch_bounds__(gemm2_cfg::NUM_THREADS, 1)
gemm2_f16_kernel(const __grid_constant__ CUtensorMap tmap_a, const __grid_constant__ CUtensorMap tmap_b,
                 const GemmParams p) {
  using namespace gemm2_cfg;
  extern __shared__ uint8_t smem_raw[];
  uint8_t* smem = reinterpret_cast<uint8_t*>((reinterpret_cast<uintptr_t>(smem_raw) + 1023) & ~uintptr_t(1023));
  uint8_t* smem_a = smem;
  uint8_t* smem_b = smem + STAGES * A_STAGE_BYTES;
  uint64_t* bars = reinterpret_cast<uint64_t*>(smem + STAGES * STAGE_BYTES);
  uint64_t* full_bar = bars;
  uint64_t* empty_bar = bars + STAGES;

  const uint32_t wg = __shfl_sync(0xffffffffu, threadIdx.x / 128, 0);
  const int tiles_m = (p.M + BLOCK_M - 1) / BLOCK_M;
  const int tiles_n = (p.N + BLOCK_N - 1) / BLOCK_N;
  const int num_tiles = tiles_m * tiles_n;
  const int num_kb1 = (p.K + BLOCK_K - 1) / BLOCK_K;
  const int num_kb = SPLIT ? 3 * num_kb1 : num_kb1;

  if (threadIdx.x == 0) {
    tma_prefetch_desc(&tmap_a);
    tma_prefetch_desc(&tmap_b);
    for (int i = 0; i < STAGES; ++i) {
      mbar_init(&full_bar[i], 1);
      mbar_init(&empty_bar[i], 2);
    }
    fence_barrier_init();
  }
  __syncthreads();
  pdl_launch_dependents();
  pdl_wait();

  if (wg == 0) {
    setmaxnreg_dec<40>();
    if (threadIdx.x == 0) {
      uint32_t it = 0;
      for (int tile = blockIdx.x; tile < num_tiles; tile += gridDim.x) {
        const int m0 = (tile / tiles_n) * BLOCK_M, n0 = (tile % tiles_n) * BLOCK_N;
        for (int kb = 0; kb < num_kb; ++kb, ++it) {
          const uint32_t s = it % STAGES;
          while (!mbar_try_wait(&empty_bar[s], ((it / STAGES) & 1) ^ 1)) __nanosleep(64);
          int a_col = kb * BLOCK_K, b_col = kb * BLOCK_K;
          if constexpr (SPLIT) {
            const int part = kb % 3;
            a_col = (kb / 3) * BLOCK_K + (part == 1 ? p.K : 0);
            b_col = (kb / 3) * BLOCK_K + (part == 2 ? p.K : 0);
          }
          mbar_arrive_expect_tx(&full_bar[s], STAGE_BYTES);
          tma_load_2d(smem_a + s * A_STAGE_BYTES, &tmap_a, &full_bar[s], a_col, m0);
          tma_load_2d(smem_b + s * B_STAGE_BYTES, &tmap_b, &full_bar[s], b_col, n0);
          tma_load_2d(smem_b + s * B_STAGE_BYTES + HALF_N * 128, &tmap_b, &full_bar[s], b_col, n0 + HALF_N);
        }
      }
    }
    return;
  }

  setmaxnreg_inc<232>();
  const uint32_t mw = wg - 1;
  const uint32_t warp = (threadIdx.x / 32) % 4;
  const uint32_t lane = threadIdx.x % 32;
  const uint32_t g = lane / 4, c = lane % 4;
  const bool signal = (threadIdx.x % 128) == 0;
  const uint32_t a_base = smem_u32(smem_a) + mw * 64 * 128;
  const uint32_t b_base = smem_u32(smem_b);
  const size_t pitch = (SPLIT && (EPI == EPI_QKV_ROPE || EPI == EPI_BIAS_GELU)) ? 2 * (size_t)p.ldo : (size_t)p.ldo;
  uint32_t it = 0;
  float acc[128];

  for (int tile = blockIdx.x; tile < num_tiles; tile += gridDim.x) {
    const int m0 = (tile / tiles_n) * BLOCK_M, n0 = (tile % tiles_n) * BLOCK_N;
    for (int kb = 0; kb < num_kb; ++kb, ++it) {
      const uint32_t s = it % STAGES;
      while (!mbar_try_wait(&full_bar[s], (it / STAGES) & 1)) {
      }
      wgmma_fence();
      const uint64_t da = wgmma_desc_sw128(a_base + s * A_STAGE_BYTES);
      const uint64_t db = wgmma_desc_sw128(b_base + s * B_STAGE_BYTES);
#pragma unroll
      for (int k = 0; k < BLOCK_K / 16; ++k) wgmma_m64n256k16(acc, da + 2 * k, db + 2 * k, (kb | k) != 0);
      wgmma_commit();
      wgmma_wait<1>();
      if (kb > 0 && signal) mbar_arrive(&empty_bar[(it + STAGES - 1) % STAGES]);
    }
    wgmma_wait<0>();
    reg_fence_f(acc);
    if (signal) mbar_arrive(&empty_bar[(it + STAGES - 1) % STAGES]);

    const int r0 = m0 + (int)(mw * 64 + warp * 16 + g);
    const int rows[2] = {r0, r0 + 8};
    if constexpr (EPI == EPI_QKV_ROPE) {
      const bool rope = p.rope_cos != nullptr;
      const int ld = p.rope_ld == 64 ? 64 : 32;
#pragma unroll
      for (int gi = 0; gi < 4; ++gi) {
        const int col0 = n0 + gi * 64;
        if (col0 >= p.N) break;
        const int sect = col0 / p.E;
        const float sc = (sect == 0) ? p.q_scale : 1.0f;
        const int slot = p.rope_ld == 64 ? ((col0 >> 6) & 1) : 0;
#pragma unroll
        for (int hr = 0; hr < 2; ++hr) {
          const int row = rows[hr];
          if (row >= p.M) continue;
          const int t = row % p.T;
          __half* o = reinterpret_cast<__half*>(p.out) + (size_t)row * pitch;
#pragma unroll
          for (int q = 0; q < 4; ++q) {
            const int j = 8 * q + 2 * (int)c;
            const float2 bl = __ldg(reinterpret_cast<const float2*>(p.bias + col0 + j));
            const float2 bh = __ldg(reinterpret_cast<const float2*>(p.bias + col0 + 32 + j));
            float a0 = (acc[4 * (8 * gi + q) + 2 * hr] + bl.x) * sc, a1 = (acc[4 * (8 * gi + q) + 2 * hr + 1] + bl.y) * sc;
            float b0 = (acc[4 * (8 * gi + q + 4) + 2 * hr] + bh.x) * sc;
            float b1 = (acc[4 * (8 * gi + q + 4) + 2 * hr + 1] + bh.y) * sc;
            if (sect < 2 && rope) {
              const float2 cs = __ldg(reinterpret_cast<const float2*>(p.rope_cos + (size_t)t * ld + slot * 32 + j));
              const float2 sn = __ldg(reinterpret_cast<const float2*>(p.rope_sin + (size_t)t * ld + slot * 32 + j));
              const float ra0 = a0 * cs.x - b0 * sn.x, rb0 = b0 * cs.x + a0 * sn.x;
              const float ra1 = a1 * cs.y - b1 * sn.y, rb1 = b1 * cs.y + a1 * sn.y;
              a0 = ra0; b0 = rb0; a1 = ra1; b1 = rb1;
            }
            const __half2 ha = __floats2half2_rn(a0, a1), hb = __floats2half2_rn(b0, b1);
            *reinterpret_cast<__half2*>(o + col0 + j) = ha;
            *reinterpret_cast<__half2*>(o + col0 + 32 + j) = hb;
            if constexpr (SPLIT) {
              const float2 fa = __half22float2(ha), fb = __half22float2(hb);
              *reinterpret_cast<__half2*>(o + p.lo_col_off + col0 + j) = __floats2half2_rn(a0 - fa.x, a1 - fa.y);
              *reinterpret_cast<__half2*>(o + p.lo_col_off + col0 + 32 + j) = __floats2half2_rn(b0 - fb.x, b1 - fb.y);
            }
          }
        }
      }
    } else {
#pragma unroll
      for (int i = 0; i < 32; ++i) {
        const int col = n0 + 8 * i + 2 * (int)c;
        if (col >= p.N) break;
        const float2 bb = __ldg(reinterpret_cast<const float2*>(p.bias + col));
#pragma unroll
        for (int hr = 0; hr < 2; ++hr) {
          const int row = rows[hr];
          if (row >= p.M) continue;
          float y0 = acc[4 * i + 2 * hr] + bb.x, y1 = acc[4 * i + 2 * hr + 1] + bb.y;
          if constexpr (EPI == EPI_BIAS_GELU || EPI == EPI_BIAS_GELU_F32) {
            y0 = gelu_erf(y0);
            y1 = gelu_erf(y1);
          }
          if constexpr (EPI == EPI_BIAS_GELU) {
            __half* o = reinterpret_cast<__half*>(p.out) + (size_t)row * pitch + col;
            const __half2 h = __floats2half2_rn(y0, y1);
            *reinterpret_cast<__half2*>(o) = h;
            if constexpr (SPLIT) {
              const float2 f = __half22float2(h);
              *reinterpret_cast<__half2*>(o + p.lo_col_off) = __floats2half2_rn(y0 - f.x, y1 - f.y);
            }
          } else {
            float2* o = reinterpret_cast<float2*>(reinterpret_cast<float*>(p.out) + (size_t)row * pitch + col);
            if constexpr (EPI == EPI_BIAS_RESIDUAL) {
              const float2 x = *o;
              *o = make_float2(x.x + y0, x.y + y1);
            } else {
              *o = make_float2(y0, y1);
            }
          }
        }
      }
    }
  }
}

template <int EPI, bool SPLIT = false>
inline cudaError_t launch_gemm2_epi(const CUtensorMap& ta, const CUtensorMap& tb, const GemmParams& p, int num_sms,
                                    cudaStream_t stream) {
  using namespace gemm2_cfg;
  cudaError_t e =
      cudaFuncSetAttribute(gemm2_f16_kernel<EPI, SPLIT>, cudaFuncAttributeMaxDynamicSharedMemorySize, SMEM_BYTES);
  if (e != cudaSuccess) return e;
  const int tiles = ((p.M + BLOCK_M - 1) / BLOCK_M) * ((p.N + BLOCK_N - 1) / BLOCK_N);
  const int grid = tiles < num_sms ? tiles : num_sms;
  return launch_pdl(gemm2_f16_kernel<EPI, SPLIT>, dim3(grid), dim3(NUM_THREADS), SMEM_BYTES, stream, ta, tb, p);
}

}
```

### esm_b200/csrc/gemm_common.cuh

```cuda
#pragma once

#include "common.cuh"

namespace esmb200 {

enum : int { EPI_QKV_ROPE = 0, EPI_BIAS_RESIDUAL = 1, EPI_BIAS_GELU = 2, EPI_BIAS_F32 = 3, EPI_BIAS_GELU_F32 = 4 };

struct GemmParams {
  int M, N, K;
  const float* bias;
  void* out;
  int ldo;
  const float* rope_cos;
  const float* rope_sin;
  int rope_ld;
  int T;
  int E;
  float q_scale;
  int lo_col_off;
};


__device__ __forceinline__ float gelu_erf(float x) {
  const float z = fabsf(x) * 0.70710678118654752440f;
  float t;
  asm("rcp.approx.ftz.f32 %0, %1;" : "=f"(t) : "f"(fmaf(0.3275911f, z, 1.0f)));
  float poly = fmaf(0.5f * 1.061405429f, t, 0.5f * -1.453152027f);
  poly = fmaf(poly, t, 0.5f * 1.421413741f);
  poly = fmaf(poly, t, 0.5f * -0.284496736f);
  poly = fmaf(poly, t, 0.5f * 0.254829592f);
  poly *= t;
  const float e = ex2_approx(z * (z * -1.4426950408889634f));
  const float q = poly * e;
  return x * (x >= 0.f ? 1.0f - q : q);
}

}
```

Baseline: 186.4.

## Stage GEMM epilogue through shared memory and write outputs with TMA store/reduce-add

Replaces direct per-thread global stores in the GEMM epilogue with stmatrix/st.shared staging into swizzled double-buffered smem boxes, then issues TMA 2D stores (or TMA reduce-add for the residual epilogue). This removes the read-modify-write of the fp32 residual and scattered half2 stores, aiming for coalesced bulk writes that overlap with the next tile's compute. It adds shared memory per CTA and named-barrier syncs per box, and makes correctness depend on the new output tensor maps.

Result: faster. 216.5, median of 6 (+16.1%).

```diff
diff --git a/esm_b200/csrc/api.cu b/esm_b200/csrc/api.cu
--- a/esm_b200/csrc/api.cu
+++ b/esm_b200/csrc/api.cu
@@ -119,6 +119,10 @@
   return make_tmap_2d(map, ptr, 2, rows, cols, ld_elems, box_rows);
 }
 
+int make_gemm_out_map(CUtensorMap* map, const void* out, int esize, uint64_t rows, uint64_t cols) {
+  return make_tmap_2d(map, out, esize, rows, cols, cols, gemm2_cfg::OUT_BOX_ROWS);
+}
+
 inline int head_slots(int E, int H) { return (H > 0 && E / H > 64) ? 2 : 1; }
 
 constexpr int kMaxDevices = 64;
@@ -149,29 +153,29 @@
 
 size_t align_up(size_t v, size_t a) { return (v + a - 1) / a * a; }
 
-int launch_gemm(int epi, const CUtensorMap& ta, const CUtensorMap& tb, const GemmParams& p, cudaStream_t st,
-                int tag = T_GEMM_OTHER, bool split = false) {
+int launch_gemm(int epi, const CUtensorMap& ta, const CUtensorMap& tb, const CUtensorMap& to, const GemmParams& p,
+                cudaStream_t st, int tag = T_GEMM_OTHER, bool split = false) {
   ProfScope ps(tag, st);
   cudaError_t e;
   if (split) {
     if (p.K % 64 != 0) return fail(ESMB200_EINVAL, "fp32x3 precision needs K % 64 == 0");
     switch (epi) {
-      case EPI_QKV_ROPE: e = launch_gemm2_epi<EPI_QKV_ROPE, true>(ta, tb, p, num_sms(), st); break;
-      case EPI_BIAS_RESIDUAL: e = launch_gemm2_epi<EPI_BIAS_RESIDUAL, true>(ta, tb, p, num_sms(), st); break;
-      case EPI_BIAS_GELU: e = launch_gemm2_epi<EPI_BIAS_GELU, true>(ta, tb, p, num_sms(), st); break;
-      case EPI_BIAS_F32: e = launch_gemm2_epi<EPI_BIAS_F32, true>(ta, tb, p, num_sms(), st); break;
-      case EPI_BIAS_GELU_F32: e = launch_gemm2_epi<EPI_BIAS_GELU_F32, true>(ta, tb, p, num_sms(), st); break;
+      case EPI_QKV_ROPE: e = launch_gemm2_epi<EPI_QKV_ROPE, true>(ta, tb, to, p, num_sms(), st); break;
+      case EPI_BIAS_RESIDUAL: e = launch_gemm2_epi<EPI_BIAS_RESIDUAL, true>(ta, tb, to, p, num_sms(), st); break;
+      case EPI_BIAS_GELU: e = launch_gemm2_epi<EPI_BIAS_GELU, true>(ta, tb, to, p, num_sms(), st); break;
+      case EPI_BIAS_F32: e = launch_gemm2_epi<EPI_BIAS_F32, true>(ta, tb, to, p, num_sms(), st); break;
+      case EPI_BIAS_GELU_F32: e = launch_gemm2_epi<EPI_BIAS_GELU_F32, true>(ta, tb, to, p, num_sms(), st); break;
       default: return fail(ESMB200_EINVAL, "unknown GEMM epilogue");
     }
     if (e != cudaSuccess) return fail_cuda(e, "gemm launch (fp32x3)");
     return ESMB200_OK;
   }
   switch (epi) {
-    case EPI_QKV_ROPE: e = launch_gemm2_epi<EPI_QKV_ROPE>(ta, tb, p, num_sms(), st); break;
-    case EPI_BIAS_RESIDUAL: e = launch_gemm2_epi<EPI_BIAS_RESIDUAL>(ta, tb, p, num_sms(), st); break;
-    case EPI_BIAS_GELU: e = launch_gemm2_epi<EPI_BIAS_GELU>(ta, tb, p, num_sms(), st); break;
-    case EPI_BIAS_F32: e = launch_gemm2_epi<EPI_BIAS_F32>(ta, tb, p, num_sms(), st); break;
-    case EPI_BIAS_GELU_F32: e = launch_gemm2_epi<EPI_BIAS_GELU_F32>(ta, tb, p, num_sms(), st); break;
+    case EPI_QKV_ROPE: e = launch_gemm2_epi<EPI_QKV_ROPE>(ta, tb, to, p, num_sms(), st); break;
+    case EPI_BIAS_RESIDUAL: e = launch_gemm2_epi<EPI_BIAS_RESIDUAL>(ta, tb, to, p, num_sms(), st); break;
+    case EPI_BIAS_GELU: e = launch_gemm2_epi<EPI_BIAS_GELU>(ta, tb, to, p, num_sms(), st); break;
+    case EPI_BIAS_F32: e = launch_gemm2_epi<EPI_BIAS_F32>(ta, tb, to, p, num_sms(), st); break;
+    case EPI_BIAS_GELU_F32: e = launch_gemm2_epi<EPI_BIAS_GELU_F32>(ta, tb, to, p, num_sms(), st); break;
     default: return fail(ESMB200_EINVAL, "unknown GEMM epilogue");
   }
   if (e != cudaSuccess) return fail_cuda(e, "gemm launch");
@@ -477,6 +481,7 @@
 
 struct ActMaps {
   CUtensorMap xn, ctx, h;
+  CUtensorMap qkv_o, h_o, x_o;
 };
 
 int layer_forward_impl(esmb200_layer* L, float* x, int B, int T, const float* rope_cos, const float* rope_sin,
@@ -494,18 +499,18 @@
   if (e != cudaSuccess) return fail_cuda(e, "layernorm1");
   GemmParams g;
   memset(&g, 0, sizeof g);
-  g.M = M; g.N = 3 * Ea; g.K = E; g.bias = L->b_qkv; g.out = ws.qkv; g.ldo = 3 * Ea;
+  g.M = M; g.N = 3 * Ea; g.K = E; g.bias = L->b_qkv;
   g.rope_cos = rope_cos; g.rope_sin = rope_sin; g.T = T; g.E = Ea; g.q_scale = L->q_scale;
   g.lo_col_off = 3 * Ea;
   g.rope_ld = 32 * L->slots;
-  int rc = launch_gemm(EPI_QKV_ROPE, am.xn, L->tm_qkv, g, st, T_QKV, split);
+  int rc = launch_gemm(EPI_QKV_ROPE, am.xn, L->tm_qkv, am.qkv_o, g, st, T_QKV, split);
   if (rc) return rc;
   rc = run_attention(ws.qkv, ws.ctx, attn_probs, attn_batch_stride, attn_flags, ws.as, B, T, H, st, split, contact,
                      L->slots);
   if (rc) return rc;
   memset(&g, 0, sizeof g);
-  g.M = M; g.N = E; g.K = Ea; g.bias = L->out_b; g.out = x; g.ldo = E;
-  rc = launch_gemm(EPI_BIAS_RESIDUAL, am.ctx, L->tm_out, g, st, T_OUT, split);
+  g.M = M; g.N = E; g.K = Ea; g.bias = L->out_b;
+  rc = launch_gemm(EPI_BIAS_RESIDUAL, am.ctx, L->tm_out, am.x_o, g, st, T_OUT, split);
   if (rc) return rc;
   {
     ProfScope ps(T_LN2, st);
@@ -514,20 +519,23 @@
   }
   if (e != cudaSuccess) return fail_cuda(e, "layernorm2");
   memset(&g, 0, sizeof g);
-  g.M = M; g.N = F; g.K = E; g.bias = L->fc1_b; g.out = ws.h; g.ldo = F; g.lo_col_off = F;
-  rc = launch_gemm(EPI_BIAS_GELU, am.xn, L->tm_fc1, g, st, T_FC1, split);
+  g.M = M; g.N = F; g.K = E; g.bias = L->fc1_b; g.lo_col_off = F;
+  rc = launch_gemm(EPI_BIAS_GELU, am.xn, L->tm_fc1, am.h_o, g, st, T_FC1, split);
   if (rc) return rc;
   memset(&g, 0, sizeof g);
-  g.M = M; g.N = E; g.K = F; g.bias = L->fc2_b; g.out = x; g.ldo = E;
-  rc = launch_gemm(EPI_BIAS_RESIDUAL, am.h, L->tm_fc2, g, st, T_FC2, split);
+  g.M = M; g.N = E; g.K = F; g.bias = L->fc2_b;
+  rc = launch_gemm(EPI_BIAS_RESIDUAL, am.h, L->tm_fc2, am.x_o, g, st, T_FC2, split);
   return rc;
 }
 
-int make_act_maps(ActMaps* am, const Workspace& ws, int E, int H, int F, int M, int split = 0) {
+int make_act_maps(ActMaps* am, const Workspace& ws, float* x, int E, int H, int F, int M, int split = 0) {
   const uint64_t Ea = (uint64_t)64 * head_slots(E, H) * H, pf = split ? 2 : 1;
   int rc = make_tmap_f16(&am->xn, ws.xn, M, pf * E, pf * E, gemm2_cfg::BOX_M);
   if (!rc) rc = make_tmap_f16(&am->ctx, ws.ctx, M, pf * Ea, pf * Ea, gemm2_cfg::BOX_M);
   if (!rc) rc = make_tmap_f16(&am->h, ws.h, M, pf * F, pf * F, gemm2_cfg::BOX_M);
+  if (!rc) rc = make_gemm_out_map(&am->qkv_o, ws.qkv, 2, M, pf * 3 * Ea);
+  if (!rc) rc = make_gemm_out_map(&am->h_o, ws.h, 2, M, pf * F);
+  if (!rc) rc = make_gemm_out_map(&am->x_o, x, 4, M, E);
   return rc;
 }
 }
@@ -562,7 +570,7 @@
   rc = carve_workspace(&ws, workspace, workspace_bytes, E, H, F, B, T, split);
   if (rc) return rc;
   ActMaps am;
-  rc = make_act_maps(&am, ws, E, H, F, B * T, split);
+  rc = make_act_maps(&am, ws, x, E, H, F, B * T, split);
   if (rc) return rc;
   rc = run_key_bits(pad_mask, ws.as, B, T, st);
   if (rc) return rc;
@@ -638,15 +646,16 @@
   if (rc) return rc;
   if (epilogue == EPI_QKV_ROPE && (!rope_cos || !rope_sin || T <= 0 || E <= 0 || E % 64 != 0 || N != 3 * E))
     return fail(ESMB200_EINVAL, "qkv epilogue needs rope tables, T and N == 3E");
-  CUtensorMap ta, tb;
+  CUtensorMap ta, tb, to;
   rc = make_tmap_f16(&ta, a, M, K, K, gemm2_cfg::BOX_M);
   if (!rc) rc = make_tmap_f16(&tb, w, N, K, K, gemm2_cfg::HALF_N);
+  if (!rc) rc = make_gemm_out_map(&to, out, f16_out ? 2 : 4, M, N);
   if (rc) return rc;
   GemmParams g;
   memset(&g, 0, sizeof g);
-  g.M = M; g.N = N; g.K = K; g.bias = bias; g.out = out; g.ldo = N;
+  g.M = M; g.N = N; g.K = K; g.bias = bias;
   g.rope_cos = rope_cos; g.rope_sin = rope_sin; g.T = T; g.E = E; g.q_scale = 0.125f;
-  return launch_gemm(epilogue, ta, tb, g, static_cast<cudaStream_t>(stream));
+  return launch_gemm(epilogue, ta, tb, to, g, static_cast<cudaStream_t>(stream));
 }
 
 int esmb200_layernorm_split(const float* x, const float* weight, const float* bias, void* out, int32_t M, int32_t E,
@@ -682,15 +691,16 @@
   if (rc) return rc;
   if (epilogue == EPI_QKV_ROPE && (!rope_cos || !rope_sin || T <= 0 || E <= 0 || E % 64 != 0 || N != 3 * E))
     return fail(ESMB200_EINVAL, "qkv epilogue needs rope tables, T and N == 3E");
-  CUtensorMap ta, tb;
+  CUtensorMap ta, tb, to;
   rc = make_tmap_f16(&ta, a, M, 2 * (uint64_t)K, 2 * (uint64_t)K, gemm2_cfg::BOX_M);
   if (!rc) rc = make_tmap_f16(&tb, w, N, 2 * (uint64_t)K, 2 * (uint64_t)K, gemm2_cfg::HALF_N);
+  if (!rc) rc = f16_out ? make_gemm_out_map(&to, out, 2, M, 2 * (uint64_t)N) : make_gemm_out_map(&to, out, 4, M, N);
   if (rc) return rc;
   GemmParams g;
   memset(&g, 0, sizeof g);
-  g.M = M; g.N = N; g.K = K; g.bias = bias; g.out = out; g.ldo = N; g.lo_col_off = N;
+  g.M = M; g.N = N; g.K = K; g.bias = bias; g.lo_col_off = N;
   g.rope_cos = rope_cos; g.rope_sin = rope_sin; g.T = T; g.E = E; g.q_scale = 0.125f;
-  return launch_gemm(epilogue, ta, tb, g, static_cast<cudaStream_t>(stream), T_GEMM_OTHER, true);
+  return launch_gemm(epilogue, ta, tb, to, g, static_cast<cudaStream_t>(stream), T_GEMM_OTHER, true);
 }
 
 int esmb200_attention_split(const void* qkv, const uint8_t* pad_mask, void* ctx, float* attn_probs, int32_t B, int32_t T,
@@ -714,15 +724,16 @@
     return fail(ESMB200_EINVAL, "rope tables must be given together with T, or not at all");
   int rc = check_device();
   if (rc) return rc;
-  CUtensorMap ta, tb;
+  CUtensorMap ta, tb, to;
   rc = make_tmap_f16(&ta, a, M, E, E, gemm2_cfg::BOX_M);
   if (!rc) rc = make_tmap_f16(&tb, w, 3 * (uint64_t)E, E, E, gemm2_cfg::HALF_N);
+  if (!rc) rc = make_gemm_out_map(&to, out, 2, M, 3 * (uint64_t)E);
   if (rc) return rc;
   GemmParams g;
   memset(&g, 0, sizeof g);
-  g.M = M; g.N = 3 * E; g.K = E; g.bias = bias; g.out = out; g.ldo = 3 * E;
+  g.M = M; g.N = 3 * E; g.K = E; g.bias = bias;
   g.rope_cos = rope_cos; g.rope_sin = rope_sin; g.T = T > 0 ? T : 1; g.E = E; g.q_scale = q_scale;
-  return launch_gemm(EPI_QKV_ROPE, ta, tb, g, static_cast<cudaStream_t>(stream));
+  return launch_gemm(EPI_QKV_ROPE, ta, tb, to, g, static_cast<cudaStream_t>(stream));
 }
 
 int esmb200_attention(const void* qkv, const uint8_t* pad_mask, void* ctx, float* attn_probs, int32_t B, int32_t T,
@@ -876,7 +887,7 @@
   uint8_t* tied_scratch = reinterpret_cast<uint8_t*>(align_up(reinterpret_cast<uintptr_t>(workspace), 1024)) + base_bytes;
   const size_t tied_bytes = esmb200_tied_row_attention_scratch_bytes(B, C, H);
   ActMaps am;
-  rc = make_act_maps(&am, ws, E, H, F, M);
+  rc = make_act_maps(&am, ws, x, E, H, F, M);
   if (rc) return rc;
   rc = run_key_bits(col_pad_mask, ws.as, B * C, R, st);
   if (rc) return rc;
@@ -895,9 +906,9 @@
     }
     if (e != cudaSuccess) return fail_cuda(e, "row layernorm");
     memset(&g, 0, sizeof g);
-    g.M = M; g.N = 3 * E; g.K = E; g.bias = L->b_qkv; g.out = ws.qkv; g.ldo = 3 * E;
+    g.M = M; g.N = 3 * E; g.K = E; g.bias = L->b_qkv;
     g.T = 1; g.E = E; g.q_scale = row_scale;
-    rc = launch_gemm(EPI_QKV_ROPE, am.xn, L->tm_qkv, g, st, T_QKV);
+    rc = launch_gemm(EPI_QKV_ROPE, am.xn, L->tm_qkv, am.qkv_o, g, st, T_QKV);
     if (rc) return rc;
     if (pad_mask) {
       ProfScope ps(T_KEYBITS, st);
@@ -908,8 +919,8 @@
                        tied_scratch, tied_bytes, stream);
     if (rc) return rc;
     memset(&g, 0, sizeof g);
-    g.M = M; g.N = E; g.K = E; g.bias = L->out_b; g.out = x; g.ldo = E;
-    rc = launch_gemm(EPI_BIAS_RESIDUAL, am.ctx, L->tm_out, g, st, T_OUT);
+    g.M = M; g.N = E; g.K = E; g.bias = L->out_b;
+    rc = launch_gemm(EPI_BIAS_RESIDUAL, am.ctx, L->tm_out, am.x_o, g, st, T_OUT);
     if (rc) return rc;
     L = col_layers[i];
     {
@@ -918,9 +929,9 @@
     }
     if (e != cudaSuccess) return fail_cuda(e, "column layernorm");
     memset(&g, 0, sizeof g);
-    g.M = M; g.N = 3 * E; g.K = E; g.bias = L->b_qkv; g.out = ws.qkv; g.ldo = 3 * E;
+    g.M = M; g.N = 3 * E; g.K = E; g.bias = L->b_qkv;
     g.T = 1; g.E = E; g.q_scale = 0.125f;
-    rc = launch_gemm(EPI_QKV_ROPE, am.xn, L->tm_qkv, g, st, T_QKV);
+    rc = launch_gemm(EPI_QKV_ROPE, am.xn, L->tm_qkv, am.qkv_o, g, st, T_QKV);
     if (rc) return rc;
     {
       AttnParams ap;
@@ -932,8 +943,8 @@
     }
     if (e != cudaSuccess) return fail_cuda(e, "column attention launch");
     memset(&g, 0, sizeof g);
-    g.M = M; g.N = E; g.K = E; g.bias = L->out_b; g.out = x; g.ldo = E;
-    rc = launch_gemm(EPI_BIAS_RESIDUAL, am.ctx, L->tm_out, g, st, T_OUT);
+    g.M = M; g.N = E; g.K = E; g.bias = L->out_b;
+    rc = launch_gemm(EPI_BIAS_RESIDUAL, am.ctx, L->tm_out, am.x_o, g, st, T_OUT);
     if (rc) return rc;
     {
       ProfScope ps(T_LN2, st);
@@ -941,12 +952,12 @@
     }
     if (e != cudaSuccess) return fail_cuda(e, "ffn layernorm");
     memset(&g, 0, sizeof g);
-    g.M = M; g.N = F; g.K = E; g.bias = L->fc1_b; g.out = ws.h; g.ldo = F;
-    rc = launch_gemm(EPI_BIAS_GELU, am.xn, L->tm_fc1, g, st, T_FC1);
+    g.M = M; g.N = F; g.K = E; g.bias = L->fc1_b;
+    rc = launch_gemm(EPI_BIAS_GELU, am.xn, L->tm_fc1, am.h_o, g, st, T_FC1);
     if (rc) return rc;
     memset(&g, 0, sizeof g);
-    g.M = M; g.N = E; g.K = F; g.bias = L->fc2_b; g.out = x; g.ldo = E;
-    rc = launch_gemm(EPI_BIAS_RESIDUAL, am.h, L->tm_fc2, g, st, T_FC2);
+    g.M = M; g.N = E; g.K = F; g.bias = L->fc2_b;
+    rc = launch_gemm(EPI_BIAS_RESIDUAL, am.h, L->tm_fc2, am.x_o, g, st, T_FC2);
     if (rc) return rc;
   }
   return ESMB200_OK;
diff --git a/esm_b200/csrc/common.cuh b/esm_b200/csrc/common.cuh
--- a/esm_b200/csrc/common.cuh
+++ b/esm_b200/csrc/common.cuh
@@ -171,6 +171,15 @@
   asm volatile("ldmatrix.sync.aligned.m8n8.x4.trans.shared.b16 {%0, %1, %2, %3}, [%4];"
                : "=r"(r[0]), "=r"(r[1]), "=r"(r[2]), "=r"(r[3])
                : "r"(addr));
+}
+
+__device__ __forceinline__ void stsm_x4(uint32_t addr, uint32_t r0, uint32_t r1, uint32_t r2, uint32_t r3) {
+  asm volatile("stmatrix.sync.aligned.m8n8.x4.shared.b16 [%0], {%1, %2, %3, %4};" ::"r"(addr), "r"(r0), "r"(r1),
+               "r"(r2), "r"(r3)
+               : "memory");
+}
+__device__ __forceinline__ void st_shared_f32x2(uint32_t addr, float a, float b) {
+  asm volatile("st.shared.v2.f32 [%0], {%1, %2};" ::"r"(addr), "f"(a), "f"(b) : "memory");
 }
 
 __device__ __forceinline__ uint32_t sw128(uint32_t base, uint32_t row, uint32_t chunk) {
diff --git a/esm_b200/csrc/gemm2.cuh b/esm_b200/csrc/gemm2.cuh
--- a/esm_b200/csrc/gemm2.cuh
+++ b/esm_b200/csrc/gemm2.cuh
@@ -14,20 +14,32 @@
 constexpr int B_STAGE_BYTES = BLOCK_N * BLOCK_K * 2;
 constexpr int STAGE_BYTES = A_STAGE_BYTES + B_STAGE_BYTES;
 constexpr int BOX_M = 128;
+constexpr int OUT_BOX_ROWS = 64;
+constexpr int OUT_BOX_BYTES = OUT_BOX_ROWS * 128;
+constexpr int OUT_BUFS = 2;
 constexpr int NUM_THREADS = 384;
-constexpr int SMEM_BYTES = STAGES * STAGE_BYTES + 1024 + 256;
+constexpr int SMEM_BYTES = STAGES * STAGE_BYTES + 2 * OUT_BUFS * OUT_BOX_BYTES + 1024 + 256;
+}
+
+__device__ __forceinline__ void stage_box_f16(uint32_t buf, uint32_t warp, uint32_t lane, const uint32_t (&h)[16]) {
+  const uint32_t m = lane / 8;
+#pragma unroll
+  for (int s = 0; s < 4; ++s)
+    stsm_x4(sw128(buf, warp * 16 + (m % 2) * 8 + lane % 8, 2 * s + m / 2), h[4 * s], h[4 * s + 1], h[4 * s + 2],
+            h[4 * s + 3]);
 }
 
 template <int EPI, bool SPLIT = false>
 __global__ void __launch_bounds__(gemm2_cfg::NUM_THREADS, 1)
 gemm2_f16_kernel(const __grid_constant__ CUtensorMap tmap_a, const __grid_constant__ CUtensorMap tmap_b,
-                 const GemmParams p) {
+                 const __grid_constant__ CUtensorMap tmap_o, const GemmParams p) {
   using namespace gemm2_cfg;
   extern __shared__ uint8_t smem_raw[];
   uint8_t* smem = reinterpret_cast<uint8_t*>((reinterpret_cast<uintptr_t>(smem_raw) + 1023) & ~uintptr_t(1023));
   uint8_t* smem_a = smem;
   uint8_t* smem_b = smem + STAGES * A_STAGE_BYTES;
-  uint64_t* bars = reinterpret_cast<uint64_t*>(smem + STAGES * STAGE_BYTES);
+  uint8_t* smem_out = smem + STAGES * STAGE_BYTES;
+  uint64_t* bars = reinterpret_cast<uint64_t*>(smem_out + 2 * OUT_BUFS * OUT_BOX_BYTES);
   uint64_t* full_bar = bars;
   uint64_t* empty_bar = bars + STAGES;
 
@@ -41,6 +53,7 @@
   if (threadIdx.x == 0) {
     tma_prefetch_desc(&tmap_a);
     tma_prefetch_desc(&tmap_b);
+    tma_prefetch_desc(&tmap_o);
     for (int i = 0; i < STAGES; ++i) {
       mbar_init(&full_bar[i], 1);
       mbar_init(&empty_bar[i], 2);
@@ -84,9 +97,25 @@
   const bool signal = (threadIdx.x % 128) == 0;
   const uint32_t a_base = smem_u32(smem_a) + mw * 64 * 128;
   const uint32_t b_base = smem_u32(smem_b);
-  const size_t pitch = (SPLIT && (EPI == EPI_QKV_ROPE || EPI == EPI_BIAS_GELU)) ? 2 * (size_t)p.ldo : (size_t)p.ldo;
+  uint8_t* const out_bufs = smem_out + mw * OUT_BUFS * OUT_BOX_BYTES;
+  uint32_t ob = 0;
   uint32_t it = 0;
   float acc[128];
+
+  auto store_box = [&](int c0, int c1) {
+    fence_proxy_async_smem();
+    if (signal) tma_store_wait_read<0>();
+    named_bar_sync(1 + mw, 128);
+    if (signal) {
+      if constexpr (EPI == EPI_BIAS_RESIDUAL) {
+        tma_reduce_add_2d(&tmap_o, out_bufs + ob * OUT_BOX_BYTES, c0, c1);
+      } else {
+        tma_store_2d(&tmap_o, out_bufs + ob * OUT_BOX_BYTES, c0, c1);
+      }
+      tma_store_commit();
+    }
+    ob ^= 1;
+  };
 
   for (int tile = blockIdx.x; tile < num_tiles; tile += gridDim.x) {
     const int m0 = (tile / tiles_n) * BLOCK_M, n0 = (tile % tiles_n) * BLOCK_N;
@@ -108,97 +137,123 @@
     if (signal) mbar_arrive(&empty_bar[(it + STAGES - 1) % STAGES]);
 
     const int r0 = m0 + (int)(mw * 64 + warp * 16 + g);
-    const int rows[2] = {r0, r0 + 8};
-    if constexpr (EPI == EPI_QKV_ROPE) {
-      const bool rope = p.rope_cos != nullptr;
-      const int ld = p.rope_ld == 64 ? 64 : 32;
+    const int box_row = m0 + (int)mw * 64;
+    if constexpr (EPI == EPI_QKV_ROPE || EPI == EPI_BIAS_GELU) {
 #pragma unroll
       for (int gi = 0; gi < 4; ++gi) {
         const int col0 = n0 + gi * 64;
         if (col0 >= p.N) break;
-        const int sect = col0 / p.E;
-        const float sc = (sect == 0) ? p.q_scale : 1.0f;
-        const int slot = p.rope_ld == 64 ? ((col0 >> 6) & 1) : 0;
-#pragma unroll
-        for (int hr = 0; hr < 2; ++hr) {
-          const int row = rows[hr];
-          if (row >= p.M) continue;
-          const int t = row % p.T;
-          __half* o = reinterpret_cast<__half*>(p.out) + (size_t)row * pitch;
+        uint32_t hi[16], lo[16];
+        if constexpr (EPI == EPI_QKV_ROPE) {
+          const int sect = col0 / p.E;
+          const float sc = (sect == 0) ? p.q_scale : 1.0f;
+          float2 bl[4], bh[4], cs[2][4], sn[2][4];
 #pragma unroll
           for (int q = 0; q < 4; ++q) {
-            const int j = 8 * q + 2 * (int)c;
-            const float2 bl = __ldg(reinterpret_cast<const float2*>(p.bias + col0 + j));
-            const float2 bh = __ldg(reinterpret_cast<const float2*>(p.bias + col0 + 32 + j));
-            float a0 = (acc[4 * (8 * gi + q) + 2 * hr] + bl.x) * sc, a1 = (acc[4 * (8 * gi + q) + 2 * hr + 1] + bl.y) * sc;
-            float b0 = (acc[4 * (8 * gi + q + 4) + 2 * hr] + bh.x) * sc;
-            float b1 = (acc[4 * (8 * gi + q + 4) + 2 * hr + 1] + bh.y) * sc;
-            if (sect < 2 && rope) {
-              const float2 cs = __ldg(reinterpret_cast<const float2*>(p.rope_cos + (size_t)t * ld + slot * 32 + j));
-              const float2 sn = __ldg(reinterpret_cast<const float2*>(p.rope_sin + (size_t)t * ld + slot * 32 + j));
-              const float ra0 = a0 * cs.x - b0 * sn.x, rb0 = b0 * cs.x + a0 * sn.x;
-              const float ra1 = a1 * cs.y - b1 * sn.y, rb1 = b1 * cs.y + a1 * sn.y;
-              a0 = ra0; b0 = rb0; a1 = ra1; b1 = rb1;
-            }
-            const __half2 ha = __floats2half2_rn(a0, a1), hb = __floats2half2_rn(b0, b1);
-            *reinterpret_cast<__half2*>(o + col0 + j) = ha;
-            *reinterpret_cast<__half2*>(o + col0 + 32 + j) = hb;
-            if constexpr (SPLIT) {
-              const float2 fa = __half22float2(ha), fb = __half22float2(hb);
-              *reinterpret_cast<__half2*>(o + p.lo_col_off + col0 + j) = __floats2half2_rn(a0 - fa.x, a1 - fa.y);
-              *reinterpret_cast<__half2*>(o + p.lo_col_off + col0 + 32 + j) = __floats2half2_rn(b0 - fb.x, b1 - fb.y);
-            }
-          }
+            bl[q] = __ldg(reinterpret_cast<const float2*>(p.bias + col0 + 8 * q + 2 * (int)c));
+            bh[q] = __ldg(reinterpret_cast<const float2*>(p.bias + col0 + 32 + 8 * q + 2 * (int)c));
+          }
+          const bool rotate = sect < 2 && p.rope_cos != nullptr;
+          if (rotate) {
+            const int ld = p.rope_ld == 64 ? 64 : 32;
+            const int slot = p.rope_ld == 64 ? ((col0 >> 6) & 1) : 0;
+#pragma unroll
+            for (int hr = 0; hr < 2; ++hr) {
+              const int t = (r0 + 8 * hr) % p.T;
+#pragma unroll
+              for (int q = 0; q < 4; ++q) {
+                const size_t at = (size_t)t * ld + slot * 32 + 8 * q + 2 * (int)c;
+                cs[hr][q] = __ldg(reinterpret_cast<const float2*>(p.rope_cos + at));
+                sn[hr][q] = __ldg(reinterpret_cast<const float2*>(p.rope_sin + at));
+              }
+            }
+          }
+#pragma unroll
+          for (int hr = 0; hr < 2; ++hr) {
+#pragma unroll
+            for (int q = 0; q < 4; ++q) {
+              float a0 = (acc[4 * (8 * gi + q) + 2 * hr] + bl[q].x) * sc;
+              float a1 = (acc[4 * (8 * gi + q) + 2 * hr + 1] + bl[q].y) * sc;
+              float b0 = (acc[4 * (8 * gi + q + 4) + 2 * hr] + bh[q].x) * sc;
+              float b1 = (acc[4 * (8 * gi + q + 4) + 2 * hr + 1] + bh[q].y) * sc;
+              if (rotate) {
+                const float2 co = cs[hr][q], si = sn[hr][q];
+                const float ra0 = a0 * co.x - b0 * si.x, rb0 = b0 * co.x + a0 * si.x;
+                const float ra1 = a1 * co.y - b1 * si.y, rb1 = b1 * co.y + a1 * si.y;
+                a0 = ra0; b0 = rb0; a1 = ra1; b1 = rb1;
+              }
+              hi[2 * q + hr] = pack_half2(a0, a1);
+              hi[2 * (q + 4) + hr] = pack_half2(b0, b1);
+              if constexpr (SPLIT) {
+                const float2 fa = __half22float2(*reinterpret_cast<const __half2*>(&hi[2 * q + hr]));
+                const float2 fb = __half22float2(*reinterpret_cast<const __half2*>(&hi[2 * (q + 4) + hr]));
+                lo[2 * q + hr] = pack_half2(a0 - fa.x, a1 - fa.y);
+                lo[2 * (q + 4) + hr] = pack_half2(b0 - fb.x, b1 - fb.y);
+              }
+            }
+          }
+        } else {
+#pragma unroll
+          for (int b = 0; b < 8; ++b) {
+            const int i = 8 * gi + b;
+            const float2 bb = __ldg(reinterpret_cast<const float2*>(p.bias + col0 + 8 * b + 2 * (int)c));
+#pragma unroll
+            for (int hr = 0; hr < 2; ++hr) {
+              const float y0 = gelu_erf(acc[4 * i + 2 * hr] + bb.x), y1 = gelu_erf(acc[4 * i + 2 * hr + 1] + bb.y);
+              hi[2 * b + hr] = pack_half2(y0, y1);
+              if constexpr (SPLIT) {
+                const float2 f = __half22float2(*reinterpret_cast<const __half2*>(&hi[2 * b + hr]));
+                lo[2 * b + hr] = pack_half2(y0 - f.x, y1 - f.y);
+              }
+            }
+          }
+        }
+        stage_box_f16(smem_u32(out_bufs + ob * OUT_BOX_BYTES), warp, lane, hi);
+        store_box(col0, box_row);
+        if constexpr (SPLIT) {
+          stage_box_f16(smem_u32(out_bufs + ob * OUT_BOX_BYTES), warp, lane, lo);
+          store_box(p.lo_col_off + col0, box_row);
         }
       }
     } else {
 #pragma unroll
-      for (int i = 0; i < 32; ++i) {
-        const int col = n0 + 8 * i + 2 * (int)c;
-        if (col >= p.N) break;
-        const float2 bb = __ldg(reinterpret_cast<const float2*>(p.bias + col));
-#pragma unroll
-        for (int hr = 0; hr < 2; ++hr) {
-          const int row = rows[hr];
-          if (row >= p.M) continue;
-          float y0 = acc[4 * i + 2 * hr] + bb.x, y1 = acc[4 * i + 2 * hr + 1] + bb.y;
-          if constexpr (EPI == EPI_BIAS_GELU || EPI == EPI_BIAS_GELU_F32) {
-            y0 = gelu_erf(y0);
-            y1 = gelu_erf(y1);
-          }
-          if constexpr (EPI == EPI_BIAS_GELU) {
-            __half* o = reinterpret_cast<__half*>(p.out) + (size_t)row * pitch + col;
-            const __half2 h = __floats2half2_rn(y0, y1);
-            *reinterpret_cast<__half2*>(o) = h;
-            if constexpr (SPLIT) {
-              const float2 f = __half22float2(h);
-              *reinterpret_cast<__half2*>(o + p.lo_col_off) = __floats2half2_rn(y0 - f.x, y1 - f.y);
-            }
-          } else {
-            float2* o = reinterpret_cast<float2*>(reinterpret_cast<float*>(p.out) + (size_t)row * pitch + col);
-            if constexpr (EPI == EPI_BIAS_RESIDUAL) {
-              const float2 x = *o;
-              *o = make_float2(x.x + y0, x.y + y1);
-            } else {
-              *o = make_float2(y0, y1);
-            }
-          }
-        }
+      for (int gi = 0; gi < 8; ++gi) {
+        const int col0 = n0 + gi * 32;
+        if (col0 >= p.N) break;
+        const uint32_t buf = smem_u32(out_bufs + ob * OUT_BOX_BYTES);
+#pragma unroll
+        for (int b = 0; b < 4; ++b) {
+          const int i = 4 * gi + b;
+          const float2 bb = col0 + 8 * b < p.N
+                                ? __ldg(reinterpret_cast<const float2*>(p.bias + col0 + 8 * b + 2 * (int)c))
+                                : make_float2(0.f, 0.f);
+#pragma unroll
+          for (int hr = 0; hr < 2; ++hr) {
+            float y0 = acc[4 * i + 2 * hr] + bb.x, y1 = acc[4 * i + 2 * hr + 1] + bb.y;
+            if constexpr (EPI == EPI_BIAS_GELU_F32) {
+              y0 = gelu_erf(y0);
+              y1 = gelu_erf(y1);
+            }
+            st_shared_f32x2(sw128(buf, warp * 16 + 8 * hr + g, 2 * b + c / 2) + (c % 2) * 8, y0, y1);
+          }
+        }
+        store_box(col0, box_row);
       }
     }
   }
+  if (signal) tma_store_wait_all();
 }
 
 template <int EPI, bool SPLIT = false>
-inline cudaError_t launch_gemm2_epi(const CUtensorMap& ta, const CUtensorMap& tb, const GemmParams& p, int num_sms,
-                                    cudaStream_t stream) {
+inline cudaError_t launch_gemm2_epi(const CUtensorMap& ta, const CUtensorMap& tb, const CUtensorMap& to,
+                                    const GemmParams& p, int num_sms, cudaStream_t stream) {
   using namespace gemm2_cfg;
   cudaError_t e =
       cudaFuncSetAttribute(gemm2_f16_kernel<EPI, SPLIT>, cudaFuncAttributeMaxDynamicSharedMemorySize, SMEM_BYTES);
   if (e != cudaSuccess) return e;
   const int tiles = ((p.M + BLOCK_M - 1) / BLOCK_M) * ((p.N + BLOCK_N - 1) / BLOCK_N);
   const int grid = tiles < num_sms ? tiles : num_sms;
-  return launch_pdl(gemm2_f16_kernel<EPI, SPLIT>, dim3(grid), dim3(NUM_THREADS), SMEM_BYTES, stream, ta, tb, p);
-}
-
-}
+  return launch_pdl(gemm2_f16_kernel<EPI, SPLIT>, dim3(grid), dim3(NUM_THREADS), SMEM_BYTES, stream, ta, tb, to, p);
+}
+
+}
diff --git a/esm_b200/csrc/gemm_common.cuh b/esm_b200/csrc/gemm_common.cuh
--- a/esm_b200/csrc/gemm_common.cuh
+++ b/esm_b200/csrc/gemm_common.cuh
@@ -9,8 +9,6 @@
 struct GemmParams {
   int M, N, K;
   const float* bias;
-  void* out;
-  int ldo;
   const float* rope_cos;
   const float* rope_sin;
   int rope_ld;
```
